# tudelft-iv/CCVPE

Hardware: AMD Instinct MI355X
Metric: image-pairs/sec (higher is better)
Workload: dtype f32

## Files before the change

ccvpe_amd/_lib.py:

```python
import ctypes
import os
import subprocess

import torch

_HERE = os.path.dirname(os.path.abspath(__file__))
LIB_PATH = os.environ.get("CCVPE_LIB") or os.path.join(_HERE, "libccvpe_hip.so")
CSRC_DIR = os.path.join(_HERE, "csrc")

c_float_p = ctypes.c_void_p
c_int = ctypes.c_int
c_float = ctypes.c_float
c_void_p = ctypes.c_void_p


class ConvDesc(ctypes.Structure):
    _fields_ = [
        ("src0", c_void_p), ("src1", c_void_p), ("gate", c_void_p), ("w", c_void_p),
        ("scale", c_void_p), ("shift", c_void_p), ("residual", c_void_p), ("dst", c_void_p),
        ("c0", c_int), ("ld0", c_int), ("c1", c_int), ("ld1", c_int),
        ("batch", c_int), ("in_h", c_int), ("in_w", c_int),
        ("kh", c_int), ("kw", c_int), ("stride", c_int), ("pad", c_int),
        ("n", c_int), ("kpad", c_int), ("ldd", c_int), ("ldres", c_int),
        ("act", c_int), ("out_mode", c_int),
    ]


class UpconvDesc(ctypes.Structure):
    _fields_ = [
        ("src0", c_void_p), ("src1", c_void_p), ("w", c_void_p), ("shift9", c_void_p), ("dst", c_void_p),
        ("c0", c_int), ("ld0", c_int), ("c1", c_int), ("ld1", c_int),
        ("batch", c_int), ("h1", c_int), ("w1", c_int),
        ("n", c_int), ("kpad", c_int), ("ldd", c_int), ("act", c_int),
    ]


class TailDesc(ctypes.Structure):
    _fields_ = [
        ("x", c_void_p), ("w", c_void_p), ("shift9", c_void_p), ("w2", c_void_p), ("b2", c_void_p), ("out", c_void_p),
        ("batch", c_int), ("h1", c_int), ("w1", c_int),
        ("c0", c_int), ("ld0", c_int), ("kpad", c_int),
        ("cout", c_int), ("normalize", c_int), ("split", c_int), ("softmax_partial", c_void_p),
    ]


PROTOTYPES = {
    "ccvpe_last_error": (ctypes.c_char_p, []),
    "ccvpe_abi_version": (c_int, []),
    "ccvpe_multi_copy_f32": (c_int, [ctypes.POINTER(c_void_p), ctypes.POINTER(c_void_p), ctypes.POINTER(c_int), c_int, c_void_p]),
    "ccvpe_gather_repack_f32": (c_int, [c_void_p, c_void_p, c_void_p, c_void_p, c_void_p, c_int, c_void_p]),
    "ccvpe_gather_repack_chunk": (c_int, []),
    "ccvpe_ctx_create": (c_int, [c_void_p, ctypes.c_longlong, c_void_p, c_void_p, ctypes.POINTER(c_void_p)]),
    "ccvpe_ctx_destroy": (c_int, [c_void_p]),
    "ccvpe_ctx_info": (c_int, [c_void_p] + [ctypes.POINTER(ctypes.c_longlong)] * 4 + [ctypes.POINTER(c_int)] * 2),
    "ccvpe_ctx_output": (c_int, [c_void_p, c_int, ctypes.POINTER(c_void_p), ctypes.POINTER(ctypes.c_longlong),
                                  ctypes.POINTER(c_int), ctypes.POINTER(ctypes.c_longlong), ctypes.POINTER(ctypes.c_longlong)]),
    "ccvpe_forward": (c_int, [c_void_p, c_void_p, c_void_p, ctypes.POINTER(c_void_p), c_void_p]),
    "ccvpe_tail512_partials": (c_int, [ctypes.POINTER(TailDesc), c_int]),
    "ccvpe_softmax_apply_f32": (c_int, [c_void_p, c_void_p, c_int, c_void_p, c_int, c_int, c_void_p]),
    "ccvpe_tail512_f32": (c_int, [ctypes.POINTER(TailDesc), c_void_p]),
    "ccvpe_tail512_bf16": (c_int, [ctypes.POINTER(TailDesc), c_void_p]),
    "ccvpe_conv_igemm_f32": (c_int, [ctypes.POINTER(ConvDesc), c_void_p]),
    "ccvpe_conv_igemm_splitk_floats": (c_int, [ctypes.POINTER(ConvDesc), c_int]),
    "ccvpe_conv_igemm_route": (c_int, [ctypes.POINTER(ConvDesc), c_int, c_int]),
    "ccvpe_set_narrow_kernels": (c_int, [c_int]),
    "ccvpe_set_pw_ring_kernels": (c_int, [c_int]),
    "ccvpe_set_mbconv_plane_kernels": (c_int, [c_int]),
    "ccvpe_mbconv_front_route": (c_int, [c_int] * 8),
    "ccvpe_mbconv_band_plan": (c_int, [c_int] * 7),
    "ccvpe_conv3x3_variant": (c_int, [ctypes.POINTER(ConvDesc), c_int]),
    "ccvpe_set_match_mfma": (c_int, [c_int]),
    "ccvpe_match_route": (c_int, [c_int, c_int, ctypes.POINTER(c_int)] + [c_int] * 10 + [ctypes.POINTER(c_int)]),
    "ccvpe_set_pwn_kernels": (c_int, [c_int]),
    "ccvpe_conv3x3_wino_ok": (c_int, [ctypes.POINTER(ConvDesc)]),
    "ccvpe_conv3x3_wino_f32": (c_int, [ctypes.POINTER(ConvDesc), c_void_p]),
    "ccvpe_conv3x3_match1_ok": (c_int, [ctypes.POINTER(ConvDesc), c_int, c_int]),
    "ccvpe_conv3x3_match1_bf16": (c_int, [ctypes.POINTER(ConvDesc), c_int, c_void_p, c_int, c_int, c_int, c_int, c_int, c_void_p, c_void_p]),
    "ccvpe_conv_igemm_splitk_f32": (c_int, [ctypes.POINTER(ConvDesc), c_void_p, c_void_p]),
    "ccvpe_conv_igemm_splitk_bf16": (c_int, [ctypes.POINTER(ConvDesc), c_int, c_void_p, c_void_p]),
    "ccvpe_upconv3x3_f32": (c_int, [ctypes.POINTER(UpconvDesc), c_void_p]),
    "ccvpe_upconv3x3_bf16": (c_int, [ctypes.POINTER(UpconvDesc), c_void_p]),
    "ccvpe_upconv3x3_route": (c_int, [ctypes.POINTER(UpconvDesc), c_int]),
    "ccvpe_upconv3x3_s3_ok": (c_int, [ctypes.POINTER(UpconvDesc)]),
    "ccvpe_upconv3x3_s3_f32": (c_int, [ctypes.POINTER(UpconvDesc), c_void_p]),
    "ccvpe_upconv3x3_s3_form_ok": (c_int, [ctypes.POINTER(UpconvDesc), c_int]),
    "ccvpe_upconv3x3_s3_route": (c_int, [ctypes.POINTER(UpconvDesc), c_int]),
    "ccvpe_upconv3x3_s3_form_f32": (c_int, [ctypes.POINTER(UpconvDesc), c_int, c_void_p]),
    "ccvpe_set_s3_quad": (c_int, [c_int]),
    "ccvpe_pw_s3_ok": (c_int, [ctypes.POINTER(ConvDesc)]),
    "ccvpe_pw_s3_route": (c_int, [ctypes.POINTER(ConvDesc)]),
    "ccvpe_pw_s3_f32": (c_int, [ctypes.POINTER(ConvDesc), c_void_p]),
    "ccvpe_stem_conv_f32": (c_int, [c_void_p] * 5 + [c_int] * 4 + [c_void_p]),
    "ccvpe_dwconv_nblk": (c_int, [c_int] * 4),
    "ccvpe_dwconv_f32": (c_int, [c_void_p] * 6 + [c_int] * 7 + [c_void_p]),
    "ccvpe_mbconv_front_nblk": (c_int, [c_int] * 6),
    "ccvpe_stem_dw_nblk": (c_int, [c_int] * 3),
    "ccvpe_stem_dw_f32": (c_int, [c_void_p] * 9 + [c_int] * 4 + [c_void_p]),
    "ccvpe_stem_dw_bf16": (c_int, [c_void_p] * 9 + [c_int] * 4 + [c_void_p]),
    "ccvpe_mbconv_front_f32": (c_int, [c_void_p, c_void_p, c_int] + [c_void_p] * 7 + [c_int] * 8 + [c_void_p]),
    "ccvpe_mbconv_front_s3_ok": (c_int, [c_int] * 7),
    "ccvpe_mbconv_front_s3_f32": (c_int, [c_void_p, c_void_p, c_int] + [c_void_p] * 7 + [c_int] * 8 + [c_void_p]),
    "ccvpe_se_gate_f32": (c_int, [c_void_p, c_int, c_float] + [c_void_p] * 5 + [c_int] * 3 + [c_void_p]),
    "ccvpe_ground_descriptor_f32": (c_int, [c_void_p, c_int, c_void_p, c_void_p, ctypes.POINTER(c_int),
                                            c_void_p, c_int, c_int, c_int, c_void_p]),
    "ccvpe_match_level_f32": (c_int, [c_void_p, c_int, c_void_p, c_int, c_int, ctypes.POINTER(c_int),
                                      c_int, c_int, c_int, c_int, c_int, c_void_p, c_void_p, c_int, c_int,
                                      c_int, c_int, c_void_p]),
    "ccvpe_head_conv3x3_f32": (c_int, [c_void_p] * 4 + [c_int] * 5 + [c_void_p]),
    "ccvpe_cast_bf16_f32": (c_int, [c_void_p, c_void_p, ctypes.c_long, c_void_p]),
    "ccvpe_softmax_rows_f32": (c_int, [c_void_p, c_void_p, c_int, c_int, c_void_p]),
    "ccvpe_eval_postprocess_f32": (c_int, [c_void_p, c_void_p, c_void_p, c_int, c_int, c_int, c_void_p]),
    "ccvpe_eval_metrics_f32": (c_int, [c_void_p] * 7 + [c_int, c_int, c_int, c_void_p]),
    "ccvpe_belief_partials": (c_int, [c_int, c_int]),
    "ccvpe_belief_step_f32": (c_int, [c_void_p] * 5 + [c_int, c_float] + [c_void_p] * 4 + [c_int] * 3 + [c_void_p]),
    "ccvpe_infonce_scratch_floats": (c_int, [c_int, c_int]),
    "ccvpe_infonce_loss_f32": (c_int, [c_void_p, c_void_p, c_float, c_void_p, c_void_p, c_void_p, c_int, c_int, c_void_p]),
    "ccvpe_cross_entropy_loss_f32": (c_int, [c_void_p] * 4 + [c_int, c_int, c_void_p]),
    "ccvpe_orientation_loss_f32": (c_int, [c_void_p] * 5 + [c_int, c_int, c_void_p]),
    "ccvpe_stem_conv_raw_f32": (c_int, [c_void_p] * 3 + [c_int] * 4 + [c_void_p]),
    "ccvpe_dwconv_raw_f32": (c_int, [c_void_p] * 3 + [c_int] * 7 + [c_void_p]),
    "ccvpe_bn_stats_nblk": (c_int, [c_int]),
    "ccvpe_bn_stats_f32": (c_int, [c_void_p, c_int, c_int] + [c_void_p] * 4 + [c_float, c_void_p, c_void_p]),
    "ccvpe_bn_act_nblk": (c_int, [c_int]),
    "ccvpe_bn_act_f32": (c_int, [c_void_p] * 5 + [c_float, c_int] + [c_void_p] * 4 + [c_int] * 3 + [c_void_p]),
    "ccvpe_conv_wgrad_tile": (c_int, [c_int, c_int]),
    "ccvpe_conv_wgrad_scratch_floats": (c_int, [c_int] * 9),
    "ccvpe_conv_wgrad_f32": (c_int, [c_void_p, c_int, c_int, c_void_p, c_int, c_int, c_void_p, c_int, c_void_p,
                                     c_void_p] + [c_int] * 8 + [c_void_p]),
    "ccvpe_conv_wgrad_gated_f32": (c_int, [c_void_p, c_int, c_int, c_void_p, c_void_p, c_int, c_void_p, c_void_p, c_int, c_int, c_int,
                                           c_int, c_void_p]),
    "ccvpe_conv_wgrad_bias_f32": (c_int, [c_void_p, c_int, c_int, c_void_p, c_int, c_int, c_void_p, c_int, c_void_p,
                                          c_void_p, c_void_p] + [c_int] * 8 + [c_void_p]),
    "ccvpe_colsum_f32": (c_int, [c_void_p, c_int, c_int, c_int, c_void_p, c_void_p, c_void_p]),
    "ccvpe_bn_bwd_nblk": (c_int, [c_int]),
    "ccvpe_bn_act_bwd_f32": (c_int, [c_void_p] * 9 + [c_float, c_int] + [c_void_p] * 4 + [c_int] * 3 + [c_void_p]),
    "ccvpe_bn_act_bwd_frozen_f32": (c_int, [c_void_p] * 9 + [c_float, c_int] + [c_void_p] * 4 + [c_int] * 3 + [c_void_p]),
    "ccvpe_se_bn_bwd_reduce_f32": (c_int, [c_void_p] * 6 + [c_float, c_int, c_void_p, c_void_p, c_int, c_int, c_int, c_void_p]),
    "ccvpe_se_bn_bwd_apply_f32": (c_int, [c_void_p] * 8 + [c_float, c_int, c_void_p, c_void_p, c_void_p, c_void_p, c_int, c_int, c_int,
                                          c_void_p]),
    "ccvpe_se_dgate_f32": (c_int, [c_void_p] * 6 + [c_float, c_int, c_void_p] + [c_int] * 3 + [c_void_p]),
    "ccvpe_se_bwd_f32": (c_int, [c_void_p, c_int, c_float, c_void_p, c_int] + [c_void_p] * 10 + [c_int] * 3 + [c_void_p]),
    "ccvpe_dwconv_dgrad_f32": (c_int, [c_void_p] * 3 + [c_int] * 7 + [c_void_p]),
    "ccvpe_dwconv_wgrad_nblk": (c_int, [c_int] * 4),
    "ccvpe_dwconv_wgrad_f32": (c_int, [c_void_p] * 4 + [c_int] * 7 + [c_void_p]),
    "ccvpe_relu_bwd_f32": (c_int, [c_void_p] * 3 + [c_int, c_void_p]),
    "ccvpe_gate_mul_f32": (c_int, [c_void_p] * 3 + [c_int] * 3 + [c_void_p]),
    "ccvpe_softmax_bwd_f32": (c_int, [c_void_p] * 4 + [c_int, c_int, c_void_p]),
    "ccvpe_l2norm2_bwd_f32": (c_int, [c_void_p] * 3 + [c_int, c_int, c_void_p]),
    "ccvpe_head_conv3x3_bwd_f32": (c_int, [c_void_p] * 7 + [c_int] * 5 + [c_void_p]),
    "ccvpe_ground_descriptor_bwd_f32": (c_int, [c_void_p, c_int, c_void_p, ctypes.POINTER(c_int)] + [c_void_p] * 4 +
                                        [c_int] * 3 + [c_void_p]),
    "ccvpe_add_cols_f32": (c_int, [c_void_p, c_int, c_int, c_void_p, c_int, c_int, c_int, c_int, c_void_p]),
    "ccvpe_stem_wgrad_nblk": (c_int, [c_int] * 3),
    "ccvpe_stem_conv_wgrad_f32": (c_int, [c_void_p] * 4 + [c_int] * 4 + [c_void_p]),
    "ccvpe_match_bwd_nblk": (c_int, [c_int, c_int, c_int]),
    "ccvpe_match_level_bwd_f32": (c_int, [c_void_p, c_int, c_void_p, c_int, c_int, ctypes.POINTER(c_int), c_int, c_int,
                                          c_int, c_int, c_int, c_void_p, c_void_p, c_void_p, c_int, c_void_p, c_int, c_void_p,
                                          c_int, c_void_p, c_int, c_int, c_int, c_void_p]),
    "ccvpe_infonce_loss_bwd_f32": (c_int, [c_void_p, c_void_p, c_float, c_void_p, c_void_p, c_void_p, c_int, c_int, c_void_p]),
    "ccvpe_cross_entropy_loss_bwd_f32": (c_int, [c_void_p] * 4 + [c_int, c_int, c_void_p]),
    "ccvpe_orientation_loss_bwd_f32": (c_int, [c_void_p] * 5 + [c_int, c_int, c_void_p]),
    "ccvpe_train_targets_nblk": (c_int, [c_int, c_int]),
    "ccvpe_train_targets_f32": (c_int, [c_void_p, c_void_p, c_int, c_float] + [c_void_p] * 10 + [c_int] * 3 + [c_void_p]),
    "ccvpe_train_targets_ordered_f32": (c_int, [c_void_p, c_void_p, c_int, c_int, c_float] + [c_void_p] * 10 + [c_int] * 3 + [c_void_p]),
    "ccvpe_adam_chunk_elems": (c_int, []),
    "ccvpe_adam_hyper_floats": (c_int, []),
    "ccvpe_adam_step_f32": (c_int, [c_void_p, c_void_p, c_void_p, c_void_p, c_int, c_float, c_void_p]),
    "ccvpe_adam_device_layout": (c_int, [c_int]),
    "ccvpe_grad_sqnorm_f32": (c_int, [c_void_p, c_void_p, c_void_p, c_int, c_float, c_void_p, c_void_p]),
    "ccvpe_adam_prepare_f32": (c_int, [c_void_p, c_void_p, c_void_p, c_void_p, c_int, c_void_p, c_int, c_float, c_void_p, c_void_p]),
    "ccvpe_adam_update_f32": (c_int, [c_void_p, c_void_p, c_void_p, c_void_p, c_int, c_float, c_void_p, c_void_p]),
    "ccvpe_preprocess_u8_f32": (c_int, [c_void_p, c_int, c_int, c_void_p, c_void_p, c_int, c_void_p, c_void_p, c_int, c_void_p,
                                        c_void_p, c_int, c_int, c_int, c_int, ctypes.POINTER(c_float), ctypes.POINTER(c_float),
                                        c_void_p]),
    "ccvpe_resize_u8": (c_int, [c_void_p, c_int, c_int, c_void_p, c_void_p, c_int, c_void_p, c_void_p, c_int, c_void_p, c_void_p,
                                c_int, c_int, c_void_p]),
    "ccvpe_gather_norm_u8_f32": (c_int, [c_void_p, c_void_p, c_int, c_int, c_int, c_int, ctypes.POINTER(c_float),
                                         ctypes.POINTER(c_float), c_void_p, c_void_p]),
    "ccvpe_window_resize_norm_u8_f32": (c_int, [c_void_p, c_int, c_int, c_void_p, c_int, c_int, c_int, c_void_p, c_void_p, c_int,
                                                c_void_p, c_void_p, c_int, ctypes.POINTER(c_float), ctypes.POINTER(c_float),
                                                c_void_p, c_int, c_int, c_void_p]),
    "ccvpe_kitti_align_u8": (c_int, [c_void_p, ctypes.c_long, c_void_p, c_void_p, c_int, c_void_p, c_int, c_int, c_void_p]),
    "ccvpe_kitti_align_norm_u8_f32": (c_int, [c_void_p, c_void_p, c_int, ctypes.POINTER(c_float), ctypes.POINTER(c_float),
                                              c_void_p, c_int, c_int, c_void_p]),
    "ccvpe_conv_igemm_bf16": (c_int, [ctypes.POINTER(ConvDesc), c_int, c_void_p]),
    "ccvpe_stem_conv_bf16": (c_int, [c_void_p] * 5 + [c_int] * 4 + [c_void_p]),
    "ccvpe_dwconv_bf16": (c_int, [c_void_p] * 6 + [c_int] * 7 + [c_void_p]),
    "ccvpe_mbconv_front_bf16": (c_int, [c_void_p, c_void_p, c_int] + [c_void_p] * 7 + [c_int] * 8 + [c_void_p]),
    "ccvpe_match_level_bf16": (c_int, [c_void_p, c_int, c_void_p, c_int, c_int, ctypes.POINTER(c_int),
                                       c_int, c_int, c_int, c_int, c_int, c_void_p, c_void_p, c_int, c_int,
                                       c_int, c_int, c_void_p]),
    "ccvpe_head_conv3x3_bf16": (c_int, [c_void_p] * 4 + [c_int] * 5 + [c_void_p]),
}

_lib = None
weights_epoch = 0


def build(verbose=False):
    cmd = ["make", "-C", CSRC_DIR, "-j8"]
    res = subprocess.run(cmd, capture_output=True, text=True)
    if verbose or res.returncode != 0:
        print(res.stdout)
        print(res.stderr)
    if res.returncode != 0:
        raise RuntimeError("building libccvpe_hip.so failed (see output above)")
    return LIB_PATH


def load():
    global _lib
    if _lib is not None:
        return _lib
    if not os.path.isfile(LIB_PATH):
        raise RuntimeError(
            "libccvpe_hip.so not found at %s — run `python -c 'import __graft_entry__ as g; g.build()'` "
            "(or `make -C ccvpe_amd/csrc`).  ccvpe_amd has no CPU fallback." % LIB_PATH)
    lib = ctypes.CDLL(LIB_PATH)
    lax = bool(os.environ.get("CCVPE_LIB")) and os.environ.get("CCVPE_LIB_ALLOW_MISSING") == "1"
    for name, (res, args) in PROTOTYPES.items():
        if lax and not hasattr(lib, name):
            continue
        fn = getattr(lib, name)
        fn.restype = res
        fn.argtypes = args
    if os.environ.get("CCVPE_NARROW") == "0" and hasattr(lib, "ccvpe_set_narrow_kernels"):
        lib.ccvpe_set_narrow_kernels(0)
    if os.environ.get("CCVPE_PW_RING") == "0" and hasattr(lib, "ccvpe_set_pw_ring_kernels"):
        lib.ccvpe_set_pw_ring_kernels(0)
    if os.environ.get("CCVPE_MATCH_MFMA") == "0" and hasattr(lib, "ccvpe_set_match_mfma"):
        lib.ccvpe_set_match_mfma(0)
    if os.environ.get("CCVPE_PWN") == "0" and hasattr(lib, "ccvpe_set_pwn_kernels"):
        lib.ccvpe_set_pwn_kernels(0)
    if os.environ.get("CCVPE_S3_QUAD") == "0" and hasattr(lib, "ccvpe_set_s3_quad"):
        lib.ccvpe_set_s3_quad(0)
    if os.environ.get("CCVPE_MBPLANE") is not None and hasattr(lib, "ccvpe_set_mbconv_plane_kernels"):
        lib.ccvpe_set_mbconv_plane_kernels(int(os.environ["CCVPE_MBPLANE"]))
    _lib = lib
    return lib


class CcvpeError(RuntimeError):
    pass


def check(status, what):
    if status != 0:
        msg = load().ccvpe_last_error()
        raise CcvpeError("%s failed (%d): %s" % (what, status, msg.decode() if msg else "?"))
```

ccvpe_amd/csrc/conv3x3_wino.hip:

```cpp
#include "conv_common.h"

namespace ccvpe {

static constexpr int WG_NW = 4;
static constexpr int WG_NT = 2;
static constexpr int WG_BN = 16 * WG_NT;
static constexpr int WG_XS = 8;
static constexpr int WG_TH = 4 * WG_NW;
static constexpr int WG_HR = WG_TH + 2, WG_HC = 18;
static constexpr int WG_HPX = WG_HR * WG_HC;
static constexpr int WG_HS = WG_HPX * LDS_LD;
static constexpr int WG_BS = 2 * WG_XS * WG_BN * 16;
static constexpr int WG_LDS = (WG_HS + WG_BS) * 4;

__global__ __launch_bounds__(256, 2) void conv3x3_wino_kernel(const IgemmParams p) {
  constexpr int NTHR = 64 * WG_NW;
  constexpr int H_IT = (WG_HPX * 4 + NTHR - 1) / NTHR;
  extern __shared__ __attribute__((aligned(16))) float wg_sm[];
  float* Hs = wg_sm;
  float* Bs = wg_sm + WG_HS;

  const int tid = threadIdx.x;
  const int lane = tid & 63;
  const int wave = sgpr(tid >> 6);
// ... 33 lines not shown
  int h_chunk = 0;
  const int ld0s = sgpr(p.ld0);
  auto load_halo = [&](int chunk) {
    h_chunk = chunk;
#pragma unroll
    for (int it = 0; it < H_IT; ++it) {
      const int ch = chunk * 16 + h_sub[it] * 4;
      const bool ok = h_pix[it] >= 0 && ch < ctot;
      const size_t off = ok ? (size_t)h_pix[it] * ld0s + ch : 0;
      h_reg[it] = *reinterpret_cast<const f32x4*>(src0 + off);
    }
  };
  auto store_halo = [&]() {
#pragma unroll
    for (int it = 0; it < H_IT; ++it)
      if (h_off[it] >= 0)
        *reinterpret_cast<f32x4*>(Hs + h_off[it]) = keep_if(h_reg[it], h_pix[it] >= 0 && h_chunk * 16 + h_sub[it] * 4 < ctot);
  };

  const int rl = lane >> 2;
  const int grp = wave & 1;
  const unsigned wvoff = ((unsigned)(n0 + grp * 16 + rl) * (unsigned)p.Kpad + (unsigned)(((lane & 3) ^ w_swz(rl)) * 4)) * 4u;
  const unsigned bs_lds = (unsigned)(uintptr_t)(__attribute__((address_space(3))) float*)Bs;
  auto load_w = [&](int chunk, int g, int dbuf) {
#pragma unroll
    for (int q = 0; q < 4; ++q) {
      const int t = (wave >> 1) + 2 * q;
      const char* sbase = reinterpret_cast<const char*>(wp) + ((size_t)(g * WG_XS + t) * cpad + (size_t)chunk * 16) * 4;
      const unsigned lds = __builtin_amdgcn_readfirstlane(bs_lds + (unsigned)(((dbuf * WG_XS + t) * WG_BN + grp * 16) * 16 * 4));
      asm volatile("s_mov_b32 m0, %0\n\tglobal_load_lds_dwordx4 %1, %2" ::"s"(lds), "v"(wvoff), "s"(sbase) : "memory", "m0");
    }
  };
  auto dma_wait = [&]() { asm volatile("s_waitcnt vmcnt(0)" ::: "memory"); };

  f32x4 acc[16][WG_NT];
#pragma unroll
  for (int x = 0; x < 16; ++x)
#pragma unroll
    for (int j = 0; j < WG_NT; ++j) acc[x][j] = (f32x4){0.f, 0.f, 0.f, 0.f};

  const int frow = lane & 15;
  const int fk = (lane >> 4) * 4;
  const int bcol = ((lane >> 4) ^ w_swz(frow)) * 4;
  const int ttx = frow & 7, tty = frow >> 3;
  const int dbase = ((4 * wave + 2 * tty) * WG_HC + 2 * ttx) * LDS_LD + fk;

  load_halo(0);
  load_w(0, 0, 0);
  store_halo();
  dma_wait();
  __syncthreads();

  int chunk = 0;
  auto stage = [&](int s, auto gtag) {
    constexpr int G = decltype(gtag)::value;
    const bool more = s + 1 < nstages;
    if (G == 0 && chunk + 1 < nchunks) load_halo(chunk + 1);
    if (more) load_w(G == 1 ? chunk + 1 : chunk, G ^ 1, (s + 1) & 1);

    f32x4 d[3][4];
#pragma unroll
    for (int r = 0; r < 3; ++r)
#pragma unroll
      for (int x = 0; x < 4; ++x) d[r][x] = *reinterpret_cast<const f32x4*>(Hs + dbase + ((G + r) * WG_HC + x) * LDS_LD);
    f32x4 v[2][4];
#pragma unroll
    for (int x = 0; x < 4; ++x) {
      const f32x4 t0 = G == 0 ? d[0][x] - d[2][x] : d[1][x] - d[0][x];
      const f32x4 t1 = G == 0 ? d[1][x] + d[2][x] : d[0][x] - d[2][x];
      if (x == 0) { v[0][0] = t0; v[1][0] = t1; }
      else if (x == 1) { v[0][1] = t0; v[1][1] = t1; }
      else if (x == 2) { v[0][2] = t0; v[1][2] = t1; }
      else { v[0][3] = t0; v[1][3] = t1; }
    }
#pragma unroll
    for (int rr = 0; rr < 2; ++rr) {
      const f32x4 a0 = v[rr][0], a1 = v[rr][1], a2 = v[rr][2], a3 = v[rr][3];
      v[rr][0] = a0 - a2;
      v[rr][1] = a1 + a2;
      v[rr][2] = a2 - a1;
      v[rr][3] = a1 - a3;
    }
    __builtin_amdgcn_sched_barrier(0);
#pragma unroll
    for (int t = 0; t < WG_XS; ++t) {
      f32x4 bf[WG_NT];
#pragma unroll
      for (int j = 0; j < WG_NT; ++j)
        bf[j] = *reinterpret_cast<const f32x4*>(&Bs[(((s & 1) * WG_XS + t) * WG_BN + j * 16 + frow) * 16 + bcol]);
      const f32x4 vv = v[t >> 2][t & 3];
#pragma unroll
      for (int kk = 0; kk < 4; ++kk)
#pragma unroll
        for (int j = 0; j < WG_NT; ++j)
          acc[G * WG_XS + t][j] = __builtin_amdgcn_mfma_f32_16x16x4f32(bf[j][kk], vv[kk], acc[G * WG_XS + t][j], 0, 0, 0);
    }
    __builtin_amdgcn_sched_barrier(0);
    dma_wait();
    __syncthreads();
    if (G == 1 && more) {
      store_halo();
      __syncthreads();
    }
  };
  for (int s = 0; s < nstages; s += 2, ++chunk) {
    stage(s, std::integral_constant<int, 0>{});
    stage(s + 1, std::integral_constant<int, 1>{});
  }

  const int oy = y0 + 4 * wave + 2 * tty, ox = x0 + 2 * ttx;
  if (oy >= p.H || ox >= p.W) return;
  float* dst = reinterpret_cast<float*>(p.dst);
  const size_t m00 = (size_t)(b * p.H + oy) * p.W + ox;
#pragma unroll
  for (int j = 0; j < WG_NT; ++j) {
    const int n = n0 + j * 16 + fk;
    if (n >= p.N) continue;
    f32x4 y[2][2];
#pragma unroll
    for (int r = 0; r < 4; ++r) {
      float m[4][4];
#pragma unroll
      for (int x = 0; x < 16; ++x) m[x >> 2][x & 3] = acc[x][j][r];
      float q0[4], q1[4];
#pragma unroll
      for (int c = 0; c < 4; ++c) {
        q0[c] = m[0][c] + m[1][c] + m[2][c];
        q1[c] = m[1][c] - m[2][c] - m[3][c];
      }
      const float bias = (p.shift && n + r < p.N) ? p.shift[n + r] : 0.0f;
      y[0][0][r] = q0[0] + q0[1] + q0[2] + bias;
      y[0][1][r] = q0[1] - q0[2] - q0[3] + bias;
      y[1][0][r] = q1[0] + q1[1] + q1[2] + bias;
      y[1][1][r] = q1[1] - q1[2] - q1[3] + bias;
    }
#pragma unroll
    for (int dy = 0; dy < 2; ++dy)
#pragma unroll
      for (int dx = 0; dx < 2; ++dx) {
        const size_t o = (m00 + (size_t)dy * p.W + dx) * p.ldd + n;
        if (n + 3 < p.N) {
          *reinterpret_cast<f32x4*>(dst + o) = y[dy][dx];
        } else {
#pragma unroll
          for (int r = 0; r < 4; ++r)
            if (n + r < p.N) dst[o + r] = y[dy][dx][r];
        }
      }
  }
}

static int round_up(int v, int m) { return (v + m - 1) / m * m; }

static const char* wino_refusal(const ccvpe_conv_desc* d) {
  if (!d) return "null desc";
  if (d->kh != 3 || d->kw != 3 || d->stride != 1 || d->pad != 1 || d->out_mode != CCVPE_OUT_NHWC) return "3x3 / stride 1 / pad 1 / NHWC only";
  if (d->c1 != 0 || d->src1 || d->gate || d->scale || d->residual || d->act != CCVPE_ACT_NONE)
    return "one source, bias only (no gate, scale, residual or activation)";
  if (d->in_h <= 0 || d->in_w <= 0 || d->in_h % 2 || d->in_w % 2) return "H and W must be even";
  if (d->c0 < 32 || d->c0 % 4 || d->ld0 < d->c0 || d->ld0 % 4) return "c0 >= 32, c0 and ld0 multiples of 4";
  if (d->n <= 0 || d->ldd < d->n || d->ldd % 4) return "ldd >= n, ldd multiple of 4";
  if (d->kpad != 16 * round_up(d->c0, 16)) return "kpad must be 16 * round_up(c0, 16) (packed U)";
  if ((long)d->batch * d->in_h * d->in_w < 16384) return "fewer than 16384 output pixels";
  if ((long)d->batch * d->in_h * d->in_w > 0x7fffffffL) return "too many pixels";
  if ((size_t)round_up(d->n, WG_BN) * d->kpad * 4 >= (1ull << 32)) return "U larger than 4 GB";
  if (!aligned16(d->src0) || !aligned16(d->w) || !aligned16(d->dst)) return "pointers must be 16-byte aligned";
  ccvpe_conv_desc dd = *d;
  dd.kpad = round_up(9 * d->c0, 16);
  if (ccvpe_conv_igemm_splitk_floats(&dd, 0) != 0) return "the direct path splits K at this shape";
  return nullptr;
}

}

using namespace ccvpe;

extern "C" int ccvpe_conv3x3_wino_ok(const ccvpe_conv_desc* d) { return wino_refusal(d) ? 0 : 1; }

extern "C" int ccvpe_conv3x3_wino_f32(const ccvpe_conv_desc* d, void* stream) {
  if (const char* why = wino_refusal(d)) return fail(CCVPE_EINVAL, "conv3x3_wino: %s", why);
  IgemmParams p{};
  p.src0 = d->src0; p.w = d->w; p.shift = d->shift; p.dst = d->dst;
  p.c0 = d->c0; p.ld0 = d->ld0;
  p.H = d->in_h; p.W = d->in_w;
  p.N = d->n; p.Kpad = d->kpad; p.Npad = round_up(d->n, WG_BN);
  p.ldd = d->ldd;
  p.tiles_x = (p.W + 15) / 16;
  p.tiles_y = (p.H + WG_TH - 1) / WG_TH;
  p.tiles_n = p.Npad / WG_BN;
  const long total = (long)p.tiles_x * p.tiles_y * d->batch * p.tiles_n;
  if (total > 0x7fffffffL) return fail(CCVPE_EINVAL, "conv3x3_wino: grid too large");
  p.tiles_total = (int)total;
  static DevCache lds_set;
  if (int rc = ensure_dyn_lds(lds_set, conv3x3_wino_kernel, WG_LDS, "conv3x3_wino")) return rc;
  hipLaunchKernelGGL(conv3x3_wino_kernel, dim3(p.tiles_total), dim3(64 * WG_NW), WG_LDS, (hipStream_t)stream, p);
  return check_launch("conv3x3_wino_kernel");
}
```

ccvpe_amd/csrc/conv_common.h:

```cpp
#pragma once
#include "common.h"
#include <cstdlib>
#include <type_traits>

namespace ccvpe {

typedef float f32x4 __attribute__((ext_vector_type(4)));
typedef __bf16 bf16_t;
typedef __bf16 bf16x8 __attribute__((ext_vector_type(8)));
typedef __bf16 bf16x4 __attribute__((ext_vector_type(4)));

template <typename T> struct ElemTraits;
template <> struct ElemTraits<float> { static constexpr int E = 4; };
template <> struct ElemTraits<bf16_t> { static constexpr int E = 8; };

template <typename T>
__device__ __forceinline__ f32x4 mfma_stage(f32x4 wfrag, f32x4 afrag, f32x4 acc);
template <>
__device__ __forceinline__ f32x4 mfma_stage<float>(f32x4 wfrag, f32x4 afrag, f32x4 acc) {
#pragma unroll
  for (int kk = 0; kk < 4; ++kk) acc = __builtin_amdgcn_mfma_f32_16x16x4f32(wfrag[kk], afrag[kk], acc, 0, 0, 0);
  return acc;
}
template <>
// ... 32 lines not shown
template <typename T>
__device__ __forceinline__ f32x4 gate_apply(f32x4 raw, f32x4 g0, f32x4 g1) {
  if (sizeof(T) == 4) return raw * g0;
  bf16x8 v = __builtin_bit_cast(bf16x8, raw);
  bf16x8 o;
#pragma unroll
  for (int i = 0; i < 4; ++i) {
    o[i] = (bf16_t)((float)v[i] * g0[i]);
    o[i + 4] = (bf16_t)((float)v[i + 4] * g1[i]);
  }
  return __builtin_bit_cast(f32x4, o);
}
__device__ __forceinline__ int sgpr(int v) { return __builtin_amdgcn_readfirstlane(v); }

struct IgemmParams {
  const void* src0;
  const void* src1;
  const float* gate;
  const void* w;
  const float* scale;
  const float* shift;
  const void* residual;
  void* dst;
  int out_f32;
  int c0, ld0, c1, ld1;
  int H, W, Ho, Wo;
  int kw, stride, pad;
  int N, Kpad, Npad;
  int cpt0, cpt, total_chunks, stages;
  int ldd, ldres, act, out_mode, cout;
  int M;
  long in_pixels;
  int tiles_n, tiles_total;
  int tiles_x, tiles_y;
  int ksplit, sps;
  float* partial;
  int ablate;
};

constexpr int LDS_LD = 20;
template <typename T> struct PanelLayout {
  static constexpr bool SWZ = true;
  static constexpr int LD = SWZ ? 16 : LDS_LD;
};
__device__ __forceinline__ int panel_swz(int row) { return ((row >> 2) & 1) << 1; }

__device__ __forceinline__ int xcd_tile(int bid, int total) {
  const int q = total / 8, r = total % 8;
  const int xcd = bid % 8, loc = bid / 8;
  return (xcd < r ? xcd * (q + 1) : r * (q + 1) + (xcd - r) * q) + loc;
}

template <typename T, int ACT>
__device__ __forceinline__ void store4(const IgemmParams& p, f32x4 v, int n, size_t obase, size_t rbase,
                                       const float* sc, const float* sh) {
#pragma unroll
  for (int r = 0; r < 4; ++r) {
    float t = v[r] * sc[r] + sh[r];
    if (ACT == CCVPE_ACT_RELU) t = fmaxf(t, 0.0f);
    else if (ACT == CCVPE_ACT_SWISH) t = swishf(t);
    v[r] = t;
  }
  const T* res = reinterpret_cast<const T*>(p.residual);
  const bool f32out = sizeof(T) == 4 || p.out_f32;
  if (n + 3 < p.N) {
    if (res) {
      f32x4 rf;
      if (sizeof(T) == 4) {
        rf = *reinterpret_cast<const f32x4*>(res + rbase + n);
      } else {
        const bf16x4 rv = *reinterpret_cast<const bf16x4*>(res + rbase + n);
#pragma unroll
        for (int r = 0; r < 4; ++r) rf[r] = (float)rv[r];
      }
      if (ACT == CCVPE_ACT_RELU_MASK) {
#pragma unroll
        for (int r = 0; r < 4; ++r) v[r] = rf[r] > 0.f ? v[r] : 0.f;
      } else {
        v += rf;
      }
    }
    if (f32out) {
      *reinterpret_cast<f32x4*>(reinterpret_cast<float*>(p.dst) + obase) = v;
    } else {
      bf16x4 o;
#pragma unroll
      for (int r = 0; r < 4; ++r) o[r] = (bf16_t)v[r];
      *reinterpret_cast<bf16x4*>(reinterpret_cast<bf16_t*>(p.dst) + obase) = o;
    }
  } else {
#pragma unroll
    for (int r = 0; r < 4; ++r)
      if (n + r < p.N) {
        float t = v[r];
        if (res) {
          const float rf = (float)res[rbase + n + r];
          t = ACT == CCVPE_ACT_RELU_MASK ? (rf > 0.f ? t : 0.f) : t + rf;
        }
        if (f32out) reinterpret_cast<float*>(p.dst)[obase + r] = t;
        else reinterpret_cast<bf16_t*>(p.dst)[obase + r] = (bf16_t)t;
      }
  }
}

#define CCVPE_ACT_DISPATCH(act, body)                                            \
  do {                                                                           \
    if ((act) == CCVPE_ACT_SWISH) body(std::integral_constant<int, CCVPE_ACT_SWISH>{});      \
    else if ((act) == CCVPE_ACT_RELU) body(std::integral_constant<int, CCVPE_ACT_RELU>{});   \
    else if ((act) == CCVPE_ACT_RELU_MASK) body(std::integral_constant<int, CCVPE_ACT_RELU_MASK>{}); \
    else body(std::integral_constant<int, CCVPE_ACT_NONE>{});                    \
  } while (0)

__device__ __forceinline__ int w_swz(int r) { return (0x1320 >> (((r >> 2) & 3) * 4)) & 3; }

#define CCVPE_TILES(X)                                                            \
  X(4, 5, 2) X(4, 4, 2) X(4, 3, 2) X(4, 2, 2) X(4, 1, 2)  \
  X(4, 5, 1) X(4, 3, 1) X(4, 1, 1)                        \
  X(2, 7, 1)

struct TileCfg { int mt, nt, wn; };
#define CCVPE_TILE_ROW(MT_, NT_, WN_) {MT_, NT_, WN_},
static const TileCfg kCfgs[] = {CCVPE_TILES(CCVPE_TILE_ROW)};
#undef CCVPE_TILE_ROW

static int pick_cfg(int npad16) {
  int best = 0;
  long best_cost = -1;
  for (int i = 0; i < (int)(sizeof(kCfgs) / sizeof(kCfgs[0])); ++i) {
    const int bn = 16 * kCfgs[i].nt * kCfgs[i].wn;
    const int tiles = (npad16 + bn - 1) / bn;
    const long cost = (long)tiles * bn * 1000 + (1000 - bn);
    if (best_cost < 0 || cost < best_cost) { best_cost = cost; best = i; }
  }
  return best;
}


template <typename T> int pw_dispatch(const IgemmParams& p, int mt, int nt, int wn, hipStream_t stream);
template <typename T> int conv3x3_dispatch(const IgemmParams& p, int batch, int mt, int nt, int wn, hipStream_t stream);
template <typename T> int conv3x3_variant_query(const IgemmParams& p, int batch, int mt, int nt, int wn);
extern bool g_use_pw2;
template <typename T> bool pw2_supported(const IgemmParams& p, int mt, int nt, int wn);
template <typename T> int pw2_dispatch(const IgemmParams& p, int mt, int nt, int wn, hipStream_t stream);
extern bool g_use_narrow;
int c3n_supported(const IgemmParams& p, int batch);
int c3n_dispatch(const IgemmParams& p, int batch, hipStream_t stream);
int c3n_match_supported(const IgemmParams& p, int batch, int L);
int c3n_match_dispatch(const IgemmParams& p, int batch, const float* g, int ldg, int L, int off, float* scores, hipStream_t stream);
extern bool g_use_pwn;
bool pwn_supported(const IgemmParams& p, int batch, int esz);
int pwn_dispatch(const IgemmParams& p, int batch, int esz, hipStream_t stream);
int up2_supported(int c0, int c1, int n, int kpad, int h1, int w1, int batch);
int up2_launch(int id, const ccvpe_upconv_desc* d, hipStream_t stream);
bool upconv_s3q_serves(const ccvpe_upconv_desc* d);
int upconv_s3q_launch(const ccvpe_upconv_desc* d, hipStream_t stream);

template <typename P>
static void s3_fill(const ccvpe_upconv_desc* d, P& p) {
  p.src0 = reinterpret_cast<const float*>(d->src0); p.src1 = reinterpret_cast<const float*>(d->src1);
  p.w = d->w; p.shift9 = d->shift9; p.dst = reinterpret_cast<float*>(d->dst);
  p.c0 = d->c0; p.ld0 = d->ld0; p.c1 = d->c1; p.ld1 = d->ld1;
  p.H1 = d->h1; p.W1 = d->w1; p.batch = d->batch; p.N = d->n; p.ldd = d->ldd; p.act = d->act;
  p.nb0 = (d->c0 + 15) / 16; p.nb1 = (d->c1 + 15) / 16; p.nst = 4 * p.nb0 + 9 * p.nb1;
}

}
```

ccvpe_amd/csrc/plan.hip:

```cpp
#include <cstring>
#include <string>
#include <unordered_map>
#include <utility>
#include <vector>

#include "common.h"

namespace ccvpe {

enum : uint32_t { K_INT = 0, K_FLT = 1, K_NULL = 2, K_WEIGHTS = 3, K_WORKSPACE = 4, K_GRD = 5, K_SAT = 6, K_STREAM = 7, K_BLOB = 8 };

template <typename A> struct FromSlot {
  static A get(uint64_t v) { return (A)(int64_t)v; }
};
template <typename P> struct FromSlot<P*> {
  static P* get(uint64_t v) { return reinterpret_cast<P*>((uintptr_t)v); }
};
template <> struct FromSlot<float> {
  static float get(uint64_t v) { uint32_t b = (uint32_t)v; float f; std::memcpy(&f, &b, 4); return f; }
};
template <typename... A, size_t... I>
static int invoke_seq(int (*f)(A...), const uint64_t* v, std::index_sequence<I...>) { return f(FromSlot<A>::get(v[I])...); }
template <typename... A>
static int invoke(int (*f)(A...), const uint64_t* v, int n) {
  if (n != (int)sizeof...(A)) return fail(CCVPE_EINVAL, "plan: call has %d arguments, the entry point takes %d", n, (int)sizeof...(A));
  return invoke_seq(f, v, std::index_sequence_for<A...>{});
}
typedef int (*Invoker)(const uint64_t*, int);

#define CCVPE_REG(fn) {#fn, [](const uint64_t* v, int n) -> int { return invoke(fn, v, n); }}
static const std::unordered_map<std::string, Invoker>& registry() {
  static const std::unordered_map<std::string, Invoker> r = {
      CCVPE_REG(ccvpe_conv_igemm_f32), CCVPE_REG(ccvpe_conv_igemm_bf16), CCVPE_REG(ccvpe_conv_igemm_splitk_f32),
      CCVPE_REG(ccvpe_conv_igemm_splitk_bf16), CCVPE_REG(ccvpe_conv3x3_match1_bf16), CCVPE_REG(ccvpe_conv3x3_wino_f32),
      CCVPE_REG(ccvpe_upconv3x3_f32), CCVPE_REG(ccvpe_upconv3x3_bf16), CCVPE_REG(ccvpe_upconv3x3_s3_f32), CCVPE_REG(ccvpe_pw_s3_f32),
      CCVPE_REG(ccvpe_tail512_f32), CCVPE_REG(ccvpe_tail512_bf16), CCVPE_REG(ccvpe_stem_conv_f32), CCVPE_REG(ccvpe_stem_conv_bf16),
      CCVPE_REG(ccvpe_stem_dw_f32), CCVPE_REG(ccvpe_stem_dw_bf16),
      CCVPE_REG(ccvpe_dwconv_f32), CCVPE_REG(ccvpe_dwconv_bf16), CCVPE_REG(ccvpe_mbconv_front_f32), CCVPE_REG(ccvpe_mbconv_front_bf16),
      CCVPE_REG(ccvpe_mbconv_front_s3_f32),
      CCVPE_REG(ccvpe_se_gate_f32), CCVPE_REG(ccvpe_ground_descriptor_f32), CCVPE_REG(ccvpe_match_level_f32),
      CCVPE_REG(ccvpe_match_level_bf16), CCVPE_REG(ccvpe_head_conv3x3_f32), CCVPE_REG(ccvpe_head_conv3x3_bf16),
      CCVPE_REG(ccvpe_softmax_rows_f32), CCVPE_REG(ccvpe_softmax_apply_f32), CCVPE_REG(ccvpe_cast_bf16_f32), CCVPE_REG(ccvpe_eval_postprocess_f32),
  };
  return r;
}
#undef CCVPE_REG

struct Patch { uint32_t call, arg, kind; uint64_t off; };
struct BlobPatch { uint32_t blob, field, kind; uint64_t off; };
struct Call { Invoker fn; std::string name; uint32_t first, nargs, sid; int wait_on; };
struct Output { uint64_t off, bytes; uint32_t dtype, ndim; long long dims[4], strides[4]; };

}

struct ccvpe_ctx {
  std::vector<ccvpe::Call> calls;
  std::vector<uint64_t> args;
  std::vector<std::vector<unsigned char>> blobs;
  std::vector<ccvpe::Patch> patches;
  std::vector<ccvpe::BlobPatch> blob_patches;
  std::vector<ccvpe::Output> outputs;
  uint64_t workspace_bytes = 0, weights_bytes = 0, grd_bytes = 0, sat_bytes = 0;
  char* weights = nullptr;
  char* workspace = nullptr;
  bool own_weights = false, own_workspace = false;
  hipStream_t side = nullptr;
  std::vector<hipEvent_t> events;
};

using namespace ccvpe;

namespace {
struct Reader {
  const unsigned char* p;
  const unsigned char* end;
  bool ok = true;
  template <typename T> T get() {
    T v{};
    if (sizeof(T) > (size_t)(end - p)) { ok = false; return v; }
    std::memcpy(&v, p, sizeof(T));
    p += sizeof(T);
    return v;
  }
  const unsigned char* bytes(size_t n) {
    if (n > (size_t)(end - p)) { ok = false; return nullptr; }
    const unsigned char* q = p;
    p += n;
    return q;
  }
};
}

extern "C" int ccvpe_ctx_create(const void* plan, long long n_bytes, void* weights_dev, void* workspace_dev, ccvpe_ctx** out) {
  if (!plan || n_bytes < 64 || !out) return fail(CCVPE_EINVAL, "ctx_create: null / short plan");
  Reader r{reinterpret_cast<const unsigned char*>(plan), reinterpret_cast<const unsigned char*>(plan) + n_bytes};
  const unsigned char* magic = r.bytes(8);
  if (!magic || std::memcmp(magic, "CCVPLAN1", 8)) return fail(CCVPE_EINVAL, "ctx_create: not a CCVPE plan (bad magic)");
  ccvpe_ctx* c = new ccvpe_ctx();
  auto bail = [&](int code, const char* msg) { delete c; return fail(code, "ctx_create: %s", msg); };
  const int abi = (int)r.get<uint32_t>();
  const uint32_t flags = r.get<uint32_t>();
  (void)flags;
  if (abi != ccvpe_abi_version()) {
    delete c;
    return fail(CCVPE_EINVAL, "ctx_create: the plan was recorded against ABI %d, this library is ABI %d", abi, ccvpe_abi_version());
  }
  c->workspace_bytes = r.get<uint64_t>();
  c->weights_bytes = r.get<uint64_t>();
  c->grd_bytes = r.get<uint64_t>();
  c->sat_bytes = r.get<uint64_t>();
  const uint32_t n_calls = r.get<uint32_t>(), n_blobs = r.get<uint32_t>(), n_out = r.get<uint32_t>();
  r.get<uint32_t>();
  if (!r.ok || n_calls > (1u << 20) || n_blobs > (1u << 20) || n_out > 64) return bail(CCVPE_EINVAL, "corrupt header");
  for (uint32_t i = 0; i < n_out; ++i) {
    Output o;
    o.off = r.get<uint64_t>(); o.bytes = r.get<uint64_t>(); o.dtype = r.get<uint32_t>(); o.ndim = r.get<uint32_t>();
    for (int k = 0; k < 4; ++k) o.dims[k] = (long long)r.get<uint64_t>();
    for (int k = 0; k < 4; ++k) o.strides[k] = (long long)r.get<uint64_t>();
    if (o.off > c->workspace_bytes || o.bytes > c->workspace_bytes - o.off) return bail(CCVPE_EINVAL, "output outside the workspace");
    c->outputs.push_back(o);
  }
  struct Reloc { uint32_t blob, field, kind; uint64_t value; };
  std::vector<Reloc> relocs;
  for (uint32_t i = 0; i < n_blobs && r.ok; ++i) {
    const uint32_t nb = r.get<uint32_t>(), nr = r.get<uint32_t>();
    for (uint32_t k = 0; k < nr; ++k) {
      Reloc q{i, r.get<uint32_t>(), r.get<uint32_t>(), r.get<uint64_t>()};
      if ((uint64_t)q.field + 8 > (uint64_t)nb) return bail(CCVPE_EINVAL, "relocation outside its blob");
      relocs.push_back(q);
    }
    const unsigned char* d = r.bytes((nb + 7) & ~7u);
    if (!d) return bail(CCVPE_EINVAL, "truncated blob");
    c->blobs.emplace_back(d, d + nb);
  }
  struct RawArg { uint32_t kind; uint64_t value; };
  std::vector<std::vector<RawArg>> raw(n_calls);
  for (uint32_t i = 0; i < n_calls && r.ok; ++i) {
    const unsigned char* nm = r.bytes(48);
    if (!nm) break;
    std::string name(reinterpret_cast<const char*>(nm), strnlen(reinterpret_cast<const char*>(nm), 48));
    const uint32_t na = r.get<uint32_t>();
    const uint32_t sid = r.get<uint32_t>() & 1u;
    if (na > 64) return bail(CCVPE_EINVAL, "call with more than 64 arguments");
    for (uint32_t k = 0; k < na; ++k) {
      RawArg a{r.get<uint32_t>(), 0};
      r.get<uint32_t>();
      a.value = r.get<uint64_t>();
      raw[i].push_back(a);
    }
    if (name == "@wait") {
      if (na != 2) return bail(CCVPE_EINVAL, "malformed stream wait");
      c->calls.push_back(Call{nullptr, name, 0, 0, (uint32_t)(raw[i][0].value & 1), (int)(raw[i][1].value & 1)});
      raw[i].clear();
      continue;
    }
    auto it = registry().find(name);
    if (it == registry().end()) {
      delete c;
      return fail(CCVPE_EINVAL, "ctx_create: the plan calls %s, which this library does not replay", name.c_str());
    }
    c->calls.push_back(Call{it->second, name, 0, na, sid, -1});
  }
  if (!r.ok) return bail(CCVPE_EINVAL, "truncated plan");
  size_t woff = (size_t)(r.p - reinterpret_cast<const unsigned char*>(plan));
  woff = (woff + 255) & ~(size_t)255;
  if (woff > (size_t)n_bytes || c->weights_bytes > (uint64_t)((size_t)n_bytes - woff)) return bail(CCVPE_EINVAL, "truncated weights");
  if (weights_dev) c->weights = reinterpret_cast<char*>(weights_dev);
  else {
    if (hipMalloc(reinterpret_cast<void**>(&c->weights), c->weights_bytes ? c->weights_bytes : 256) != hipSuccess) return bail(CCVPE_ELAUNCH, "hipMalloc(weights)");
    c->own_weights = true;
  }
  if (workspace_dev) c->workspace = reinterpret_cast<char*>(workspace_dev);
  else {
    if (hipMalloc(reinterpret_cast<void**>(&c->workspace), c->workspace_bytes ? c->workspace_bytes : 256) != hipSuccess) {
      if (c->own_weights) (void)hipFree(c->weights);
      return bail(CCVPE_ELAUNCH, "hipMalloc(workspace)");
    }
    c->own_workspace = true;
  }
  if (c->weights_bytes &&
      hipMemcpy(c->weights, reinterpret_cast<const unsigned char*>(plan) + woff, c->weights_bytes, hipMemcpyHostToDevice) != hipSuccess) {
    ccvpe_ctx_destroy(c);
    return fail(CCVPE_ELAUNCH, "ctx_create: weight upload failed");
  }
  auto resolve = [&](uint32_t kind, uint64_t v, bool& dynamic, bool& bad) -> uint64_t {
    dynamic = bad = false;
    switch (kind) {
// ... 108 lines not shown
```

ccvpe_amd/models.py:

```python
import torch
import torch.nn as nn

from . import ops
from .synth import B0_BLOCKS, MODEL_SPECS, state_dict_spec

BN_EPS = 1e-3
SKIP_BLOCKS = (15, 10, 4, 2, 0)
MATCH_STRIDES = {"vigor": (64, 32, 16, 8, 4, 2),
                 "kitti": (128, 64, 32, 16, 8, 8),
                 "oxford": (64, 32, 16, 8, 4, 2)}


def window_offset(kind, channels, length):
    return int(channels / 2 - length / 2) if kind == "oxford" else 0


def _round_up(v, m):
    return (v + m - 1) // m * m


class _Holder(nn.Module):

    def forward(self, *a, **k):
        raise RuntimeError("parameter holder is not callable; use the owning CVM_* module")


def _populate(root, kind, init):
    for key, shape, role in state_dict_spec(kind):
        parts = key.split(".")
        node = root
        for name in parts[:-1]:
            child = node._modules.get(name)
            if child is None:
                child = _Holder()
                node.add_module(name, child)
            node = child
        t = init[key].clone()
        if role in ("bn_m", "bn_v", "bn_n"):
            node.register_buffer(parts[-1], t)
        else:
            node.register_parameter(parts[-1], nn.Parameter(t))


def _pad2(w, dtype=torch.float32, n_mult=16):
    k_mult = 16 if dtype == torch.float32 else 32
    n, k = w.shape
    if n % n_mult == 0 and k % k_mult == 0:
        out = w.to(dtype).contiguous()
        return out.clone() if out.data_ptr() == w.data_ptr() else out
    out = w.new_zeros((_round_up(n, n_mult), _round_up(k, k_mult)))
    out[:n, :k] = w
    return out.to(dtype).contiguous()


def _pack_conv(w, dtype=torch.float32):
    o = w.shape[0]
    return _pad2(w.permute(0, 2, 3, 1).reshape(o, -1), dtype)


_WINO_G = ((1.0, 0.0, 0.0), (0.5, 0.5, 0.5), (0.5, -0.5, 0.5), (0.0, 0.0, 1.0))


def _pack_wino(w, dtype=torch.float32):
    if dtype != torch.float32:
        return None
    o, i = w.shape[0], w.shape[1]
    g = torch.tensor(_WINO_G, dtype=torch.float64, device=w.device)
    u = torch.einsum("ak,ockl,bl->oabc", g, w.to(torch.float64), g)
    out = torch.zeros((_round_up(o, 32), 4, 4, _round_up(i, 16)), dtype=torch.float64, device=w.device)
    out[:o, :, :, :i] = u
    return out.reshape(out.shape[0], -1).to(torch.float32).contiguous()


def _fold_bn(sd, p):
    scale = sd[p + ".weight"] / torch.sqrt(sd[p + ".running_var"] + BN_EPS)
    shift = sd[p + ".bias"] - sd[p + ".running_mean"] * scale
    return scale.contiguous(), shift.contiguous()


class _Obj(object):
    pass


def _pack_pw_s3(w):
    if w is None or w.dtype != torch.float32 or w.dim() != 2 or w.shape[1] % 16 or w.shape[0] % 16:
        return None
    npad, k = w.shape
    return torch.cat(_split3_bf16(w.reshape(npad, k // 16, 16).permute(1, 0, 2)), -1).contiguous()


def _unpack_pw_s3(w3):
    nst, npad, _ = w3.shape
    return tuple(w3[..., 16 * q:16 * q + 16].float().permute(1, 0, 2).reshape(npad, nst * 16) for q in range(3))


PW_S3_MIN_MID = 240


MB_S3_MAX_CIN = 48


def _pack_encoder(sd, p, dtype=torch.float32, fold_bn=True, s3=False):
    fold = _fold_bn if fold_bn else (lambda _sd, _p: (None, None))
    e = _Obj()
    e.stem_w = sd[p + "._conv_stem.weight"].permute(2, 3, 1, 0).contiguous()
    e.stem_scale, e.stem_shift = fold(sd, p + "._bn0")
    e.blocks = []
    for i, (k, s, ex, cin, cout) in enumerate(B0_BLOCKS):
        b = _Obj()
        bp = "%s._blocks.%d" % (p, i)
        b.k, b.s, b.expand, b.cin, b.cout, b.mid = k, s, ex != 1, cin, cout, cin * ex
        if b.expand:
            b.w_exp = _pack_conv(sd[bp + "._expand_conv.weight"], dtype)
            b.s0, b.b0 = fold(sd, bp + "._bn0")
            b.w_exp3 = _pack_pw_s3(b.w_exp) if s3 and cin <= MB_S3_MAX_CIN else None
        b.w_dw = sd[bp + "._depthwise_conv.weight"].reshape(b.mid, k, k).permute(1, 2, 0).contiguous()
        b.s1, b.b1 = fold(sd, bp + "._bn1")
        b.se_w1 = sd[bp + "._se_reduce.weight"].reshape(-1, b.mid).contiguous()
        b.se_b1 = sd[bp + "._se_reduce.bias"].contiguous()
        b.se_w2 = sd[bp + "._se_expand.weight"].reshape(b.mid, -1).t().contiguous()
        b.se_b2 = sd[bp + "._se_expand.bias"].contiguous()
        b.w_proj = _pack_conv(sd[bp + "._project_conv.weight"], dtype)
        b.w_proj3 = _pack_pw_s3(b.w_proj) if s3 and b.mid >= PW_S3_MIN_MID else None
        b.s2, b.b2 = fold(sd, bp + "._bn2")
        b.skip = (s == 1 and cin == cout)
        e.blocks.append(b)
    e.w_head = _pack_conv(sd[p + "._conv_head.weight"], dtype)
    e.w_head3 = _pack_pw_s3(e.w_head) if s3 else None
    e.head_scale, e.head_shift = fold(sd, p + "._bn1")
    return e


def _pack_deconv(w, bias, col_map, ldo, dtype=torch.float32):
    cin, cout = w.shape[0], w.shape[1]
    wg = w.permute(2, 3, 1, 0).reshape(4 * cout, cin)
    out = w.new_zeros((4 * cout, ldo))
    for d0, s0, n in col_map:
        out[:, d0:d0 + n] = wg[:, s0:s0 + n]
    return _pad2(out, dtype), bias.repeat(4).contiguous()


_UP_S = {0: {0: ((0, 1),), 1: ((1, 0), (2, 1))}, 1: {0: ((0, 0), (1, 1)), 1: ((2, 0),)}}
_UP_R = {0: (1, 2), 1: (0, 1, 2), 2: (0, 1)}
_OVERLAP_ENV = __import__("os").environ.get("CCVPE_OVERLAP_DECODERS", "auto")


OVERLAP_DECODERS_MAX_BATCH = 128


def _overlap_decoders(precision, batch=1):
    return _OVERLAP_ENV == "1" or (_OVERLAP_ENV == "auto" and precision == "bf16" and batch <= OVERLAP_DECODERS_MAX_BATCH)
FOLD_LEVELS = tuple(int(c) for c in __import__("os").environ.get("CCVPE_FOLD_LEVELS", "012345"))
FOLD_MIN_PIXELS = int(__import__("os").environ.get("CCVPE_FOLD_MIN_PIXELS", "2048"))
FUSE_TAIL = __import__("os").environ.get("CCVPE_FUSE_TAIL", "1") != "0"
SPLIT_TAIL = __import__("os").environ.get("CCVPE_SPLIT_TAIL", "1") != "0"
WINO = __import__("os").environ.get("CCVPE_WINO", "1") != "0"
SPLIT3 = __import__("os").environ.get("CCVPE_SPLIT3", "1") != "0"
SPLIT3_TAIL = SPLIT3 and __import__("os").environ.get("CCVPE_SPLIT3_TAIL", "1") != "0"
SPLIT3_MIN_OK = 2
SPLIT3_PW = SPLIT3 and __import__("os").environ.get("CCVPE_SPLIT3_PW", "1") != "0"
SPLIT3_PW_MIN_OK = 2
SPLIT3_MB = SPLIT3 and __import__("os").environ.get("CCVPE_SPLIT3_MB", "1") != "0"
SPLIT3_MB_MIN_OK = 2
PACK_GRAPH = __import__("os").environ.get("CCVPE_PACK_GRAPH", "1") != "0"
PACK_GATHER = __import__("os").environ.get("CCVPE_PACK_GATHER", "1") != "0"
FUSE_MATCH = __import__("os").environ.get("CCVPE_FUSE_MATCH", "1") != "0"
FUSE_STEM = __import__("os").environ.get("CCVPE_FUSE_STEM", "1") != "0"
EVAL_TWO_STREAMS = __import__("os").environ.get("CCVPE_EVAL_TWO_STREAMS", "1") != "0"


def _tail_split(precision, x, cout):
    if x.dtype != torch.float32:
        return 0
    if precision == "bf16":
        return 1 if SPLIT_TAIL and cout == 1 else 0
    return 2 if SPLIT3 and SPLIT3_TAIL else 0


def _pack_upconv(wd, bd, col_map, cp, w3, b3, dtype=torch.float32):
    cd, co = wd.shape[1], w3.shape[0]
    c1 = w3.shape[1] - cd
    wd_my = wd.new_zeros((cp, cd, 2, 2), dtype=torch.float64)
    for d0, s0, n in col_map:
        wd_my[d0:d0 + n] = wd[s0:s0 + n].double()
    w3d = w3[:, :cd].double()
    k = 4 * cp + 9 * c1
    kmult = 16 if dtype == torch.float32 else 32
    out = wd.new_zeros((4, _round_up(co, 16), _round_up(k, kmult)), dtype=torch.float64)
    for py in range(2):
        for px in range(2):
            par = py * 2 + px
            for du in range(2):
                for dv in range(2):
                    weff = wd.new_zeros((co, cp), dtype=torch.float64)
                    for ky, a in _UP_S[py][du]:
                        for kx, b in _UP_S[px][dv]:
                            weff += w3d[:, :, ky, kx] @ wd_my[:, :, a, b].t()
                    tap = du * 2 + dv
                    out[par, :co, tap * cp:(tap + 1) * cp] = weff
            if c1:
                out[par, :co, 4 * cp:k] = w3[:, cd:].double().permute(0, 2, 3, 1).reshape(co, 9 * c1)
    shift9 = wd.new_zeros((9, co), dtype=torch.float64)
    for rc in range(3):
        for cc in range(3):
            v = b3.double().clone()
            for ky in _UP_R[rc]:
                for kx in _UP_R[cc]:
                    v += w3d[:, :, ky, kx] @ bd.double()
            shift9[rc * 3 + cc] = v
    return out.to(dtype).contiguous(), shift9.float().contiguous()


def _split3_bf16(v):
    hi = v.to(torch.bfloat16)
    r = v - hi.float()
    mid = r.to(torch.bfloat16)
    lo = (r - mid.float()).to(torch.bfloat16)
    return hi, mid, lo


def _pack_upconv_s3(fw, cp, c1, dtype=torch.float32):
    if dtype != torch.float32 or fw is None or fw.dtype != torch.float32 or c1 <= 0:
        return None
    npad = fw.shape[1]
    nb0, nb1 = (cp + 15) // 16, (c1 + 15) // 16
    a = fw.new_zeros((4, npad, 4, nb0 * 16))
    a[..., :cp] = fw[:, :, :4 * cp].reshape(4, npad, 4, cp)
    a = a.reshape(4, npad, 4, nb0, 16).permute(0, 3, 2, 1, 4).reshape(4, 4 * nb0, npad, 16)
    s = fw.new_zeros((4, npad, 9, nb1 * 16))
    s[..., :c1] = fw[:, :, 4 * cp:4 * cp + 9 * c1].reshape(4, npad, 9, c1)
    s = s.reshape(4, npad, 9, nb1, 16).permute(0, 2, 3, 1, 4).reshape(4, 9 * nb1, npad, 16)
    return torch.cat(_split3_bf16(torch.cat([a, s], 1)), -1).contiguous()


def _pack_backward(sd, kind, pk):
    spec = MODEL_SPECS[kind]
    n_rot = spec["n_rot"]
    bwd = {}
    for enc in ("grd_efficientnet", "sat_efficientnet"):
        for i, (k, s_, ex, cin, cout) in enumerate(B0_BLOCKS):
            bp = "%s._blocks.%d" % (enc, i)
            if ex != 1:
                bwd[bp + "._expand_conv.weight"] = _pack_conv(sd[bp + "._expand_conv.weight"].permute(1, 0, 2, 3))
            bwd[bp + "._project_conv.weight"] = _pack_conv(sd[bp + "._project_conv.weight"].permute(1, 0, 2, 3))
            if s_ == 1:
                mid = cin * ex
                w_dw = sd[bp + "._depthwise_conv.weight"].reshape(mid, k * k).t()
                bwd[bp + "._depthwise_conv.weight"] = w_dw.flip(0).contiguous()
        bwd[enc + "._conv_head.weight"] = _pack_conv(sd[enc + "._conv_head.weight"].permute(1, 0, 2, 3))
    for j in range(6):
        lvl = 6 - j
        for branch, lv in (("", pk.loc[j]), ("_ori", pk.ori[j])):
            conv, deconv = "conv%d%s" % (lvl, branch), "deconv%d%s" % (lvl, branch)
            if lvl != 1:
                bwd[conv + ".2.weight"] = _pack_conv(sd[conv + ".2.weight"].flip(2, 3).permute(1, 0, 2, 3))
            bwd[conv + ".0.weight"] = _pack_conv(sd[conv + ".0.weight"].flip(2, 3).permute(1, 0, 2, 3))
            w_ref = sd[deconv + ".weight"]
            if branch == "":
                c = lv.c
                k_rows, cmap = lv.ldo, [(0, 1, c), (c, 0, 1)]
            elif j == 0:
                c6 = spec["ori"][0][0] - n_rot
                k_rows, cmap = lv.k, [(0, n_rot, c6), (c6 + 1, 0, n_rot)]
            else:
                k_rows, cmap = lv.k, [(0, 0, spec["ori"][j][0])]
            w_ours = w_ref.new_zeros((k_rows,) + tuple(w_ref.shape[1:]))
            for d0, s0, n in cmap:
                w_ours[d0:d0 + n] = w_ref[s0:s0 + n]
            bwd[deconv + ".weight"] = _pack_conv(w_ours)
    w = sd["sat_feature_to_descriptors.1.weight"]
    w4 = w.view(w.shape[0], 1280, 2, 2)
    bwd["sat_feature_to_descriptors.1.weight"] = _pack_deconv(w4, w4.new_zeros((1280,)), [(0, 0, w.shape[0])], w.shape[0])[0]
    wcat = torch.cat([sd["grd_feature_to_descriptor%d.0.weight" % l] for l in range(1, 7)], 0)
    ld = _round_up(pk.gd_n, 4)
    wpad = wcat.new_zeros((ld,) + tuple(wcat.shape[1:]))
    wpad[:pk.gd_n] = wcat
    bwd["grd_feature_to_descriptor.0.weight"] = _pack_conv(wpad.permute(1, 0, 2, 3))
    return bwd


def _pack_model(sd, kind, n_tail, dtype=torch.float32, fold=True, f32_tail=0):
    spec = MODEL_SPECS[kind]
    pk = _Obj()
    pk.dtype = dtype
    pk.f32_from = 6 - f32_tail if dtype != torch.float32 else 6
    base_dtype = dtype
    s3 = fold and dtype == torch.float32
    pk.grd = _pack_encoder(sd, "grd_efficientnet", dtype, fold_bn=fold, s3=s3)
    pk.sat = _pack_encoder(sd, "sat_efficientnet", dtype, fold_bn=fold, s3=s3)
    ws, bs, wh, bh = [], [], [], []
    for l in range(1, 7):
        p = "grd_feature_to_descriptor%d" % l
        ws.append(sd[p + ".0.weight"].reshape(-1, 1280))
        bs.append(sd[p + ".0.bias"])
        wh.append(sd[p + ".2.weight"].reshape(-1))
        bh.append(sd[p + ".2.bias"].reshape(-1))
    pk.gd_w = _pad2(torch.cat(ws, 0), dtype)
    pk.gd_w3 = _pack_pw_s3(pk.gd_w) if s3 else None
    pk.gd_bias = torch.cat(bs, 0).contiguous()
    pk.gd_n = pk.gd_bias.shape[0]
    pk.gd_wh = torch.stack(wh, 0).contiguous()
    pk.gd_bh = torch.cat(bh, 0).contiguous()
    w = sd["sat_feature_to_descriptors.1.weight"]
    pk.sd_w = _pack_conv(w.view(w.shape[0], 1280, 2, 2), dtype)
    pk.sd_w3 = _pack_pw_s3(pk.sd_w) if s3 else None
    pk.sd_bias = sd["sat_feature_to_descriptors.1.bias"].contiguous()
    pk.sd_n = w.shape[0]

    pk.loc, pk.ori = [], []
    n_rot = spec["n_rot"]
    for j in range(6):
        lvl = 6 - j
        dc_in, dc_out, c_in, c_out = spec["loc"][j]
        dtype = torch.float32 if j >= pk.f32_from else base_dtype
        c = dc_in - 1
        ldo = _round_up(c + 1 + (n_tail if j == 0 else 0), 8)
        lv = _Obj()
        lv.c, lv.ldo, lv.up_n = c, ldo, 4 * dc_out
        lv.up_w, lv.up_b = _pack_deconv(sd["deconv%d.weight" % lvl], sd["deconv%d.bias" % lvl],
                                        [(0, 1, c), (c, 0, 1)], ldo, dtype)
        lv.c0, lv.c1 = dc_out, c_in - dc_out
        lv.n_a = c_out
        if fold and j in FOLD_LEVELS:
            lv.fw, lv.fshift = _pack_upconv(sd["deconv%d.weight" % lvl], sd["deconv%d.bias" % lvl],
                                            [(0, 1, c), (c, 0, 1)], ldo, sd["conv%d.0.weight" % lvl],
                                            sd["conv%d.0.bias" % lvl], dtype)
            lv.fw3 = _pack_upconv_s3(lv.fw, ldo, lv.c1, dtype if base_dtype == torch.float32 else None)
        lv.w_a = _pack_conv(sd["conv%d.0.weight" % lvl], dtype)
        lv.b_a = sd["conv%d.0.bias" % lvl].contiguous()
        if lvl != 1:
            lv.w_b = _pack_conv(sd["conv%d.2.weight" % lvl], dtype)
            lv.u_b = _pack_wino(sd["conv%d.2.weight" % lvl], base_dtype) if fold else None
            lv.n_b = c_out
        else:
            lv.w_b = sd["conv1.2.weight"].permute(0, 2, 3, 1).contiguous()
        lv.b_b = sd["conv%d.2.bias" % lvl].contiguous()
        pk.loc.append(lv)
        dtype = base_dtype
        dc_in, dc_out, c_in, c_out = spec["ori"][j]
        ov = _Obj()
        if j == 0:
            c6 = dc_in - n_rot
            ov.k = pk.loc[0].ldo
            ov.k_algo = dc_in
            ov.up_w, ov.up_b = _pack_deconv(sd["deconv6_ori.weight"], sd["deconv6_ori.bias"],
                                            [(0, n_rot, c6), (c6 + 1, 0, n_rot)], pk.loc[0].ldo, dtype)
        else:
            ov.k = ov.k_algo = dc_in
            ov.up_w, ov.up_b = _pack_deconv(sd["deconv%d_ori.weight" % lvl], sd["deconv%d_ori.bias" % lvl],
                                            [(0, 0, dc_in)], dc_in, dtype)
        ov.up_n = 4 * dc_out
        ov.c0, ov.c1 = dc_out, c_in - dc_out
        if fold and j in FOLD_LEVELS:
            cmap = [(0, n_rot, c6), (c6 + 1, 0, n_rot)] if j == 0 else [(0, 0, dc_in)]
            ov.fw, ov.fshift = _pack_upconv(sd["deconv%d_ori.weight" % lvl], sd["deconv%d_ori.bias" % lvl], cmap,
                                            ov.k, sd["conv%d_ori.0.weight" % lvl], sd["conv%d_ori.0.bias" % lvl],
                                            dtype)
            ov.fw3 = _pack_upconv_s3(ov.fw, ov.k, ov.c1, dtype)
        ov.w_a = _pack_conv(sd["conv%d_ori.0.weight" % lvl], dtype)
        ov.b_a = sd["conv%d_ori.0.bias" % lvl].contiguous()
        ov.n_a = c_out
        if lvl != 1:
            ov.w_b = _pack_conv(sd["conv%d_ori.2.weight" % lvl], dtype)
            ov.u_b = _pack_wino(sd["conv%d_ori.2.weight" % lvl], dtype) if fold else None
            ov.n_b = c_out
        else:
            ov.w_b = sd["conv1_ori.2.weight"].permute(0, 2, 3, 1).contiguous()
        ov.b_b = sd["conv%d_ori.2.bias" % lvl].contiguous()
        pk.ori.append(ov)
    pk.bwd = _pack_backward(sd, kind, pk) if (not fold and base_dtype == torch.float32) else None
    return pk


def _pw(x, c0, w, w3, n, *, batch, in_h, in_w, two=False, gate=None, scale=None, shift=None, residual=None, act=ops.ACT_NONE,
        ldd=None, out_f32=False):
    if (SPLIT3 and SPLIT3_PW and w3 is not None and x.dtype == torch.float32 and
            ops.pw_s3_ok(x, c0, w3, n, batch=batch, in_h=in_h, in_w=in_w, two=two, gate=gate, residual=residual, act=act,
                         ldd=ldd) >= SPLIT3_PW_MIN_OK):
        return ops.pw_s3(x, c0, w3, n, batch=batch, in_h=in_h, in_w=in_w, two=two, gate=gate, scale=scale, shift=shift,
                         residual=residual, act=act, ldd=ldd)
    kk = dict(kh=2, kw=2, stride=2) if two else {}
    return ops.conv_igemm(x, c0, w, n, batch=batch, in_h=in_h, in_w=in_w, gate=gate, scale=scale, shift=shift, residual=residual,
                          act=act, ldd=ldd, out_f32=out_f32, **kk)


def _run_encoder(e, img, circular, multiscale, dtype=torch.float32):
    blk0 = e.blocks[0]
    stem_fused = (FUSE_STEM and not blk0.expand and blk0.k == 3 and blk0.s == 1 and blk0.mid == 32
                  and ops.stem_dw_supported(img.shape[2], img.shape[3], circular) > 0)
    x = None if stem_fused else ops.stem_conv(img, e.stem_w, e.stem_scale, e.stem_shift, circular, out_dtype=dtype)
    feats = []
    for blk in e.blocks:
        if x is not None:
            b, h, w, _ = x.shape
        if x is None:
            u, part = ops.stem_dw(img, e.stem_w, e.stem_scale, e.stem_shift, blk.w_dw, blk.s1, blk.b1, circular,
                                  out_dtype=dtype)
            b = u.shape[0]
        elif blk.expand and ops.mbconv_front_supported(h, w, blk.cin, blk.mid, blk.k, blk.s):
            w3 = getattr(blk, "w_exp3", None)
            if SPLIT3 and SPLIT3_MB and w3 is not None and ops.mbconv_front_s3_ok(x, w3, blk.mid, blk.k, blk.s) >= SPLIT3_MB_MIN_OK:
                u, part = ops.mbconv_front_s3(x, w3, blk.s0, blk.b0, blk.w_dw, blk.s1, blk.b1, blk.mid, blk.k, blk.s, circular)
            else:
                u, part = ops.mbconv_front(x, blk.w_exp, blk.s0, blk.b0, blk.w_dw, blk.s1, blk.b1, blk.mid,
                                           blk.k, blk.s, circular)
        else:
            t = x
            if blk.expand:
                t = ops.conv_igemm(x, blk.cin, blk.w_exp, blk.mid, batch=b, in_h=h, in_w=w,
                                   scale=blk.s0, shift=blk.b0, act=ops.ACT_SWISH)
            u, part = ops.dwconv(t, blk.w_dw, blk.s1, blk.b1, blk.k, blk.s, circular)
        ho, wo = u.shape[1], u.shape[2]
        gate = ops.se_gate(part, ho * wo, blk.se_w1, blk.se_b1, blk.se_w2, blk.se_b2)
        x = _pw(u, blk.mid, blk.w_proj, getattr(blk, "w_proj3", None), blk.cout, batch=b, in_h=ho, in_w=wo, gate=gate,
                scale=blk.s2, shift=blk.b2, residual=x if blk.skip else None)
        if multiscale:
            feats.append(x)
    b, h, w, _ = x.shape
    f = _pw(x, 320, e.w_head, getattr(e, "w_head3", None), 1280, batch=b, in_h=h, in_w=w, scale=e.head_scale,
            shift=e.head_shift, act=ops.ACT_SWISH)
    return f, feats


def _double_conv(lv, up, skip, batch, hw):
    y = ops.conv_igemm(up, lv.c0, lv.w_a, lv.n_a, batch=batch, in_h=hw, in_w=hw, kh=3, kw=3, pad=1,
                       src1=skip, c1=lv.c1, shift=lv.b_a, act=ops.ACT_RELU)
    return y


def _conv_b(lv, y, batch, hw, out_f32=False):
    if (WINO and lv.u_b is not None and
            ops.conv3x3_wino_ok(y, lv.n_a, lv.u_b, lv.n_b, batch=batch, in_h=hw, in_w=hw)):
        return ops.conv3x3_wino(y, lv.n_a, lv.u_b, lv.n_b, batch=batch, in_h=hw, in_w=hw, shift=lv.b_b)
    return ops.conv_igemm(y, lv.n_a, lv.w_b, lv.n_b, batch=batch, in_h=hw, in_w=hw, kh=3, kw=3, pad=1, shift=lv.b_b,
                          out_f32=out_f32)


def _upconv_a(lv, x, k, batch, hw, skip):
    fw3 = getattr(lv, "fw3", None)
    if (SPLIT3 and fw3 is not None and
            ops.upconv3x3_s3_ok(x, k, fw3, lv.n_a, batch=batch, h1=hw, w1=hw, src1=skip, c1=lv.c1) >= SPLIT3_MIN_OK):
        return ops.upconv3x3_s3(x, k, fw3, lv.fshift, lv.n_a, batch=batch, h1=hw, w1=hw, src1=skip, c1=lv.c1, act=ops.ACT_RELU)
    return ops.upconv3x3(x, k, lv.fw, lv.fshift, lv.n_a, batch=batch, h1=hw, w1=hw, src1=skip, c1=lv.c1, act=ops.ACT_RELU)


class _CVMBase(nn.Module):
    kind = "vigor"

    def __init__(self, device, circular_padding, ori_noise=None, efficientnet_weights=None):
        super().__init__()
        self.device = device
        self.circular_padding = circular_padding
        self.ori_noise = ori_noise
        from . import init as _init
        _populate(self, self.kind, _init.reference_init_state_dict(self.kind))
        weights = efficientnet_weights if efficientnet_weights is not None else __import__("os").environ.get("CCVPE_EFFICIENTNET_B0")
        if weights:
            _init.load_efficientnet_b0(self, weights)
        self._pack_cache = None
        self._pack_key = None
        self.precision = "fp32"
        self.fp32_tail_levels = 1

    def set_precision(self, precision, fp32_tail_levels=1):
        if precision not in ("fp32", "bf16"):
            raise ValueError("precision must be 'fp32' or 'bf16'")
        if not 0 <= int(fp32_tail_levels) <= 5:
            raise ValueError("fp32_tail_levels must be in 0..5 (level 6 feeds the bf16 orientation decoder)")
        self.precision = precision
        self.fp32_tail_levels = int(fp32_tail_levels)
        return self

    def invalidate(self):
        self._pack_cache = None
        self._pack_key = None
        object.__setattr__(self, "_flat_tensors", None)
        return self

    def _weights_key(self):
        from . import _lib
        flat = getattr(self, "_flat_tensors", None)
        if flat is None:
            flat = list(self.parameters()) + list(self.buffers())
            object.__setattr__(self, "_flat_tensors", flat)
        return (_lib.weights_epoch,) + tuple((t.data_ptr(), t._version) for t in flat)

    def _packed(self):
        epoch = 0 if self.training else getattr(self, "_stats_epoch", 0)
        key = (self.precision, self.fp32_tail_levels, self.training, epoch) + self._weights_key()
        if self._pack_cache is not None and key == self._pack_key:
            return self._pack_cache
        dev = next(self.parameters()).device
        if dev.type != "cuda":
            raise RuntimeError("ccvpe_amd: move the model to the MI355X first (.to('cuda'))")
        sd = {k: v.detach() for k, v in self.state_dict().items()}
        n_tail = MODEL_SPECS[self.kind]["n_rot"]
        dtype = torch.float32 if self.precision == "fp32" else torch.bfloat16

        def pack(src=sd):
            with torch.no_grad():
                return _pack_model(src, self.kind, n_tail, dtype, fold=not self.training, f32_tail=self.fp32_tail_levels)

        if self.training and PACK_GATHER and dtype == torch.float32 and not getattr(self, "_pack_plan_failed", False):
            from . import repack
            where = tuple(t.data_ptr() for t in list(self.parameters()) + list(self.buffers()))
            gp = getattr(self, "_pack_plan", None)
            if gp is not None and gp[0] == where:
                self._pack_cache = gp[1].run()
            else:
                plan = repack.build(sd, pack)
                if plan is None:
                    self._pack_plan, self._pack_plan_failed = None, True
                    return self._packed()
                self._pack_plan = (where, plan)
                self._pack_cache = plan.pk
        elif self.training and PACK_GRAPH:
            where = (self.precision, self.fp32_tail_levels) + tuple(
                t.data_ptr() for t in list(self.parameters()) + list(self.buffers()))
            g = getattr(self, "_pack_graph", None)
            if g is not None and g[0] == where:
                g[1].replay()
                self._pack_cache = g[2]
            elif getattr(self, "_pack_where", None) == where and not getattr(self, "_pack_graph_failed", False):
                try:
                    graph = torch.cuda.CUDAGraph()
                    with torch.cuda.graph(graph, capture_error_mode="thread_local"):
                        pk = pack()
                    graph.replay()
                    self._pack_graph = (where, graph, pk)
                    self._pack_cache = pk
                except Exception:
                    self._pack_graph, self._pack_graph_failed = None, True
                    self._pack_cache = pack()
            else:
                self._pack_graph = None
                self._pack_where = where
                self._pack_cache = pack()
        else:
            self._pack_cache = pack()
        self._pack_key = key
        return self._pack_cache

    def _side_stream(self, which=1):
        dev = next(self.parameters()).device
        streams = self.__dict__.setdefault("_side_streams", {})
        st = streams.get(which)
        if st is None or st.device != dev:
            st = torch.cuda.Stream(device=dev)
            streams[which] = st
        return st

    def _ori_decoder(self, pk, cat6, sfeats, batch):
        xo = cat6
        normalize = not getattr(self, "ori_raw_output", False)
        for j in range(6):
            ov = pk.ori[j]
            hw = xo.shape[1]
            skip = sfeats[SKIP_BLOCKS[j]] if j < 5 else None
            if j == 5 and FUSE_TAIL and j in FOLD_LEVELS and ops.tail512_ok(hw, hw, ov.n_a):
                return ops.tail512(xo, ov.k, ov.fw, ov.fshift, ov.w_b, ov.b_b, 2, normalize, batch=batch, h1=hw, w1=hw,
                                   split=_tail_split(self.precision, xo, 2))
            if j in FOLD_LEVELS and batch * hw * hw >= FOLD_MIN_PIXELS:
                y = _upconv_a(ov, xo, ov.k, batch, hw, skip)
            else:
                up = ops.conv_igemm(xo, ov.k, ov.up_w, ov.up_n, batch=batch, in_h=hw, in_w=hw,
                                    shift=ov.up_b, out_mode=ops.OUT_DECONV2X, algo_k=ov.k_algo)
                y = _double_conv(ov, up, skip, batch, 2 * hw)
            if j < 5:
                xo = _conv_b(ov, y, batch, 2 * hw)
            else:
                return ops.head_conv3x3(y, ov.w_b, ov.b_b, 2, normalize)

    def _loc_shifts(self):
        n_rot = MODEL_SPECS[self.kind]["n_rot"]
        if self.ori_noise is None:
            return list(range(n_rot))
        k = int(self.ori_noise / 18)
        return list(range(-k, k + 1))

    drop_connect_rate = 0.2
    BN_MOMENTUM = 0.01

    bn_frozen = False

    def freeze_batchnorm(self, mode=True):
        self.bn_frozen = bool(mode)
        return self

    def forward(self, grd, sat, drop_masks=None):
        if self.training and self.precision != "fp32":
            raise NotImplementedError("ccvpe_amd: train mode is fp32 only")
        if not (grd.is_cuda and sat.is_cuda):
            raise RuntimeError("ccvpe_amd runs on the MI355X only: inputs must be device tensors")
        if self.training:
            from . import train
            if torch.is_grad_enabled() and any(p.requires_grad for p in self.parameters()):
                outs = train.apply(self, grd, sat, drop_masks)
            else:
                with torch.no_grad():
                    outs, _ = train.forward_train(self, grd, sat, drop_masks, rec=False)
            outs = list(outs)
            if self.ori_noise is not None:
                outs[3] = outs[3][:, len(self._loc_shifts()):]
            return tuple(outs)
        main = torch.cuda.current_stream()
        return self._forward_eval(grd, sat, main, self._side_stream() if EVAL_TWO_STREAMS else main)

    def _forward_eval(self, grd, sat, main, side):
        spec = MODEL_SPECS[self.kind]
        n_rot = spec["n_rot"]
        strides = MATCH_STRIDES[self.kind]
        circular = bool(self.circular_padding) and self.kind == "vigor"
        with torch.no_grad():
            pk = self._packed()
            grd = grd.contiguous().float()
            sat = sat.contiguous().float()
            batch = grd.shape[0]

            side.wait_stream(main)
            with torch.cuda.stream(side):
                gfeat, _ = _run_encoder(pk.grd, grd, circular, False, pk.dtype)
                _, gh, gw, _ = gfeat.shape
                if gh != spec["grd_h"]:
                    raise ValueError("ground feature height %d != %d expected by the descriptor heads"
                                     % (gh, spec["grd_h"]))
                y1 = _pw(gfeat, 1280, pk.gd_w, pk.gd_w3, pk.gd_n, batch=batch, in_h=gh, in_w=gw,
                         shift=pk.gd_bias, ldd=_round_up(pk.gd_n, 4), out_f32=True)
                gdesc = ops.ground_descriptor(y1, pk.gd_wh, pk.gd_bh, spec["cd"])
            svol, sfeats = _run_encoder(pk.sat, sat, False, True, pk.dtype)
            main.wait_stream(side)
            gdesc.record_stream(main)
            sdesc = _pw(svol, 1280, pk.sd_w, pk.sd_w3, pk.sd_n, batch=batch, in_h=svol.shape[1],
                        in_w=svol.shape[2], two=True, shift=pk.sd_bias)

            overlap = _overlap_decoders(self.precision, batch)
            loc_shifts = self._loc_shifts()
            fused = None
            scores_out = []
            smx = None
            x = sdesc
            cat6 = None
            goff = 0
            sfeats_loc = sfeats
            for j in range(6):
                lv = pk.loc[j]
                if j == pk.f32_from:
                    x = ops.cast_f32(x)
                    sfeats_loc = dict((SKIP_BLOCKS[q], ops.cast_f32(sfeats[SKIP_BLOCKS[q]])) for q in range(j, 5))
                hw = x.shape[1]
                cd = spec["cd"][j]
                L = gw * cd
                g = gdesc[:, goff:goff + L]
                goff += L
                if j == 0:
                    if self.ori_noise is None:
                        shifts, n_max = list(range(n_rot)), n_rot
                    else:
                        shifts, n_max = loc_shifts + list(range(n_rot)), len(loc_shifts)
                    n_tail = n_rot
                else:
                    shifts, n_max, n_tail = loc_shifts, len(loc_shifts), 0
                if fused is not None:
                    sc, cat = fused
                    fused = None
                else:
                    sc, cat = ops.match_level(x, g, L, shifts, n_max, n_tail, strides[j], lv.ldo, channels=lv.c,
                                              window_offset=window_offset(self.kind, lv.c, L))
                if j == 0:
                    cat6 = cat
                    scores_out.append(sc if self.ori_noise is None else sc[:, n_max:])
                    if overlap:
                        side.wait_stream(main)
                        with torch.cuda.stream(side):
                            x_ori = self._ori_decoder(pk, cat6, sfeats, batch)
                else:
                    scores_out.append(sc)
                skip = sfeats_loc[SKIP_BLOCKS[j]] if j < 5 else None
                if j == 5 and FUSE_TAIL and j in FOLD_LEVELS and ops.tail512_ok(hw, hw, lv.n_a):
                    logits_map, smx = ops.tail512(cat, lv.ldo, lv.fw, lv.fshift, lv.w_b, lv.b_b, 1, False, batch=batch, h1=hw, w1=hw,
                                                  split=_tail_split(self.precision, cat, 1),
                                                  want_softmax=True)
                    break
                if j in FOLD_LEVELS and batch * hw * hw >= FOLD_MIN_PIXELS:
                    y = _upconv_a(lv, cat, lv.ldo, batch, hw, skip)
                else:
                    up = ops.conv_igemm(cat, lv.ldo, lv.up_w, lv.up_n, batch=batch, in_h=hw, in_w=hw,
                                        shift=lv.up_b, out_mode=ops.OUT_DECONV2X, algo_k=lv.c + 1)
                    y = _double_conv(lv, up, skip, batch, 2 * hw)
                if j < 5:
                    to_f32 = j + 1 == pk.f32_from and y.dtype != torch.float32
                    nxt = pk.loc[j + 1]
                    L_n = gw * spec["cd"][j + 1]
                    if (FUSE_MATCH and len(loc_shifts) == 1 and
                            ops.conv3x3_match1(y, lv.n_a, lv.w_b, lv.n_b, None, L_n, loc_shifts[0], strides[j + 1], nxt.ldo, batch=batch,
                                               in_h=2 * hw, in_w=2 * hw, bias=lv.b_b, out_f32=to_f32, query_only=True)):
                        fused = ops.conv3x3_match1(y, lv.n_a, lv.w_b, lv.n_b, gdesc[:, goff:goff + L_n], L_n, loc_shifts[0],
                                                   strides[j + 1], nxt.ldo, batch=batch, in_h=2 * hw, in_w=2 * hw, bias=lv.b_b,
                                                   window_offset=window_offset(self.kind, nxt.c, L_n), out_f32=to_f32)
                        x = fused[1]
                    else:
                        x = _conv_b(lv, y, batch, 2 * hw, out_f32=to_f32)
                else:
                    logits_map = ops.head_conv3x3(y, lv.w_b, lv.b_b, 1, False)
            logits = logits_map.reshape(batch, -1)
            if smx is not None:
                heatmap = ops.softmax_apply(logits, smx).reshape(logits_map.shape)
            else:
                heatmap = ops.softmax_rows(logits).reshape(logits_map.shape)

            if overlap:
                main.wait_stream(side)
                x_ori.record_stream(main)
            else:
                x_ori = self._ori_decoder(pk, cat6, sfeats, batch)
        return (logits, heatmap, x_ori) + tuple(scores_out)


class CVM_VIGOR(_CVMBase):
    kind = "vigor"

    def __init__(self, device, circular_padding, efficientnet_weights=None):
        super().__init__(device, circular_padding, None, efficientnet_weights)


class CVM_VIGOR_ori_prior(_CVMBase):
    kind = "vigor"

    def __init__(self, device, ori_noise, circular_padding=True, efficientnet_weights=None):
        super().__init__(device, circular_padding, ori_noise, efficientnet_weights)


class CVM_OxfordRobotCar(_CVMBase):
    kind = "oxford"

    def __init__(self, device, efficientnet_weights=None):
        super().__init__(device, False, None, efficientnet_weights)


class CVM_KITTI(_CVMBase):
    kind = "kitti"

    def __init__(self, device, efficientnet_weights=None):
        super().__init__(device, False, None, efficientnet_weights)
```

ccvpe_amd/ops.py:

```python
import ctypes

import torch

from . import _lib
from ._lib import ConvDesc, check

ACT_NONE, ACT_RELU, ACT_SWISH, ACT_RELU_MASK = 0, 1, 2, 3
SPLIT_K_CALLS = 0
SPLIT_K = __import__("os").environ.get("CCVPE_SPLIT_K", "1") == "1"
OUT_NHWC, OUT_DECONV2X = 0, 1

_recorder = None


def set_recorder(rec):
    global _recorder
    _recorder = rec


class LaunchRecorder(object):

    def __init__(self):
        self.items = []

# ... 88 lines not shown
    return "%s_f32_kernel<%d,%d,%d>" % (fam, mt, nt, wn)


_record = None


def _empty(shape, device=None, dtype=torch.float32):
    if _record is not None:
        return _record.empty(shape, dtype, device)
    return torch.empty(shape, device=device, dtype=dtype)


def _ptr(t):
    if t is None:
        return None
    if _record is not None:
        _record.note(t)
    return ctypes.c_void_p(t.data_ptr())


def _chk(t, name, dtype=torch.float32):
    if t is None:
        return
    if not t.is_cuda or t.dtype != dtype or not t.is_contiguous():
        raise ValueError("%s must be a contiguous %s device tensor (got %s %s contiguous=%s)" % (
            name, dtype, t.device, t.dtype, t.is_contiguous()))


def _act_dtype(t):
    if t.dtype not in (torch.float32, torch.bfloat16):
        raise ValueError("activations must be fp32 or bf16, got %s" % t.dtype)
    return t.dtype


def conv_igemm(src0, c0, w_packed, n, *, batch, in_h, in_w, kh=1, kw=1, stride=1, pad=0,
               src1=None, c1=0, gate=None, scale=None, shift=None, residual=None, act=ACT_NONE,
               out_mode=OUT_NHWC, dst=None, ldd=None, ld0=None, ld1=None, algo_k=None, out_f32=False, route_only=False,
               variant_only=False):
    lib = _lib.load()
    dt = _act_dtype(src0)
    odt = torch.float32 if (out_f32 or dt == torch.float32) else dt
    for t, nm in ((src0, "src0"), (src1, "src1"), (w_packed, "w"), (residual, "residual")):
        _chk(t, nm, dt)
    for t, nm in ((gate, "gate"), (scale, "scale"), (shift, "shift")):
        _chk(t, nm)
    _chk(dst, "dst", odt)
    ld0 = ld0 if ld0 is not None else src0.shape[-1]
    ld1 = ld1 if ld1 is not None else (src1.shape[-1] if src1 is not None else 0)
    ho = (in_h + 2 * pad - kh) // stride + 1
    wo = (in_w + 2 * pad - kw) // stride + 1
    if out_mode == OUT_DECONV2X:
        cout = n // 4
        oshape = (batch, 2 * ho, 2 * wo)
    else:
        cout = n
        oshape = (batch, ho, wo)
    if dst is None:
        ldd = ldd if ldd is not None else cout
        dst = _empty(oshape + (ldd,), device=src0.device, dtype=odt)
    elif ldd is None:
        ldd = dst.shape[-1]
    d = ConvDesc()
    d.src0, d.src1, d.gate, d.w = _ptr(src0), _ptr(src1), _ptr(gate), _ptr(w_packed)
    d.scale, d.shift, d.residual, d.dst = _ptr(scale), _ptr(shift), _ptr(residual), _ptr(dst)
    d.c0, d.ld0, d.c1, d.ld1 = c0, ld0, c1, ld1
    d.batch, d.in_h, d.in_w = batch, in_h, in_w
    d.kh, d.kw, d.stride, d.pad = kh, kw, stride, pad
    d.n, d.kpad = n, w_packed.shape[1]
    d.ldd = ldd
    d.ldres = residual.shape[-1] if residual is not None else 0
    d.act, d.out_mode = act, out_mode
    if route_only:
        return conv_route(d, dt != torch.float32, bool(out_f32))
    if variant_only:
        return conv3x3_variant(d, dt != torch.float32)
    rec = _recorder
    ev0 = rec.begin() if rec is not None else None
    want = lib.ccvpe_conv_igemm_splitk_floats(ctypes.byref(d), int(dt != torch.float32)) if SPLIT_K else 0
    if want < 0:
        check(int(want), "ccvpe_conv_igemm_splitk_floats")
    if want > 0:
        global SPLIT_K_CALLS
        SPLIT_K_CALLS += 1
        scratch = _empty((want,), device=src0.device, dtype=torch.float32)
        if dt == torch.float32:
            check(lib.ccvpe_conv_igemm_splitk_f32(ctypes.byref(d), _ptr(scratch), _stream()), "ccvpe_conv_igemm_splitk_f32")
        else:
            check(lib.ccvpe_conv_igemm_splitk_bf16(ctypes.byref(d), int(bool(out_f32)), _ptr(scratch), _stream()),
                  "ccvpe_conv_igemm_splitk_bf16")
    elif dt == torch.float32:
        check(lib.ccvpe_conv_igemm_f32(ctypes.byref(d), _stream()), "ccvpe_conv_igemm_f32")
    else:
        check(lib.ccvpe_conv_igemm_bf16(ctypes.byref(d), int(bool(out_f32)), _stream()), "ccvpe_conv_igemm_bf16")
    if rec is not None:
        m = batch * ho * wo
        k_alg = algo_k if algo_k is not None else kh * kw * (c0 + c1)
        flops = 2.0 * m * n * k_alg
        esz = 4.0 if dt == torch.float32 else 2.0
        nbytes = esz * (batch * in_h * in_w * (c0 + c1) + m * n + n * k_alg
                        + (m * n if residual is not None else 0))
        if want > 0:
            name = igemm_tile(n, False)
        else:
            name = conv_route_name(d, dt != torch.float32, bool(out_f32))
        if want > 0 and dt != torch.float32:
            name = name.replace("_f32_kernel<", "_kernel<bf16,")
        rec.end(name, "%dx%d s%d M%d N%d K%d" % (kh, kw, stride, m, n, k_alg), flops, nbytes, ev0)
    return dst


def _wino_desc(src0, c0, u_packed, n, batch, in_h, in_w, shift, dst, ldd, ld0):
    d = ConvDesc()
    d.src0, d.src1, d.gate, d.w = _ptr(src0), None, None, _ptr(u_packed)
    d.scale, d.shift, d.residual, d.dst = None, _ptr(shift), None, _ptr(dst) if dst is not None else None
    d.c0, d.ld0, d.c1, d.ld1 = c0, ld0, 0, 0
    d.batch, d.in_h, d.in_w = batch, in_h, in_w
    d.kh, d.kw, d.stride, d.pad = 3, 3, 1, 1
    d.n, d.kpad = n, u_packed.shape[1]
    d.ldd, d.ldres = ldd, 0
    d.act, d.out_mode = ACT_NONE, OUT_NHWC
    return d


def conv3x3_wino_ok(src0, c0, u_packed, n, *, batch, in_h, in_w, ldd=None, ld0=None):
    if src0.dtype != torch.float32 or u_packed is None:
        return False
    ld0 = ld0 if ld0 is not None else src0.shape[-1]
    d = _wino_desc(src0, c0, u_packed, n, batch, in_h, in_w, None, None, ldd if ldd is not None else n, ld0)
    return bool(_lib.load().ccvpe_conv3x3_wino_ok(ctypes.byref(d)))


def conv3x3_wino(src0, c0, u_packed, n, *, batch, in_h, in_w, shift=None, dst=None, ldd=None, ld0=None):
    lib = _lib.load()
    for t, nm in ((src0, "src0"), (u_packed, "w"), (shift, "shift"), (dst, "dst")):
        _chk(t, nm)
    ld0 = ld0 if ld0 is not None else src0.shape[-1]
    if dst is None:
        ldd = ldd if ldd is not None else n
        dst = _empty((batch, in_h, in_w, ldd), device=src0.device)
    elif ldd is None:
        ldd = dst.shape[-1]
    d = _wino_desc(src0, c0, u_packed, n, batch, in_h, in_w, shift, dst, ldd, ld0)
    rec = _recorder
    ev0 = rec.begin() if rec is not None else None
    check(lib.ccvpe_conv3x3_wino_f32(ctypes.byref(d), _stream()), "ccvpe_conv3x3_wino_f32")
    if rec is not None:
        m = batch * in_h * in_w
        flops = 2.0 * m * n * 9 * c0
        nbytes = 4.0 * (m * c0 + m * n + n * 9 * c0)
        rec.end("conv3x3_wino_f32_kernel<16x16,32>", "3x3 s1 M%d N%d K%d" % (m, n, 9 * c0), flops, nbytes, ev0)
    return dst


def upconv3x3(src0, c0, w_packed, shift9, n, *, batch, h1, w1, src1=None, c1=0, act=ACT_NONE, algo_flops=None, route_only=False):
    lib = _lib.load()
    dt = _act_dtype(src0)
    for t, nm in ((src0, "src0"), (src1, "src1"), (w_packed, "w")):
        _chk(t, nm, dt)
    _chk(shift9, "shift9")
    dst = _empty((batch, 2 * h1, 2 * w1, n), device=src0.device, dtype=dt)
    d = _lib.UpconvDesc()
    d.src0, d.src1, d.w, d.shift9, d.dst = _ptr(src0), _ptr(src1), _ptr(w_packed), _ptr(shift9), _ptr(dst)
    d.c0, d.ld0, d.c1, d.ld1 = c0, src0.shape[-1], c1, (src1.shape[-1] if src1 is not None else 0)
    d.batch, d.h1, d.w1 = batch, h1, w1
    d.n, d.kpad, d.ldd, d.act = n, w_packed.shape[-1], n, act
    if route_only:
        return upconv_route(d, dt != torch.float32)
    rec = _recorder
    ev0 = rec.begin() if rec is not None else None
    fn = lib.ccvpe_upconv3x3_f32 if dt == torch.float32 else lib.ccvpe_upconv3x3_bf16
    check(fn(ctypes.byref(d), _stream()), "ccvpe_upconv3x3")
    if rec is not None:
        m = batch * h1 * w1 * 4
        k_eff = 4 * c0 + 9 * c1
        flops = algo_flops if algo_flops is not None else 2.0 * m * n * k_eff
        esz = 4.0 if dt == torch.float32 else 2.0
        nbytes = esz * (batch * h1 * w1 * c0 + m * c1 + m * n + 4 * n * k_eff)
        name = upconv_route_name(d, dt != torch.float32)
        rec.end(name, "up3x3 M%d N%d Keff%d" % (m, n, k_eff), flops, nbytes, ev0)
    return dst


def _s3_desc(src0, c0, w3_packed, shift9, n, batch, h1, w1, src1, c1, act, dst, ldd, ld0, ld1):
    d = _lib.UpconvDesc()
    d.src0, d.src1, d.w, d.shift9 = _ptr(src0), _ptr(src1), _ptr(w3_packed), _ptr(shift9)
    d.dst = _ptr(dst) if dst is not None else None
    d.c0, d.ld0, d.c1, d.ld1 = c0, ld0, c1, ld1
    d.batch, d.h1, d.w1 = batch, h1, w1
    d.n, d.kpad, d.ldd, d.act = n, w3_packed.shape[1] * w3_packed.shape[3], ldd, act
    return d


def upconv3x3_s3_ok(src0, c0, w3_packed, n, *, batch, h1, w1, src1=None, c1=0, ldd=None, ld0=None, ld1=None):
    if w3_packed is None or src0.dtype != torch.float32 or (src1 is not None and src1.dtype != torch.float32):
        return 0
    if w3_packed.dtype != torch.bfloat16 or w3_packed.dim() != 4:
        return 0
    ld0 = ld0 if ld0 is not None else src0.shape[-1]
    ld1 = ld1 if ld1 is not None else (src1.shape[-1] if src1 is not None else 0)
    d = _s3_desc(src0, c0, w3_packed, None, n, batch, h1, w1, src1, c1, ACT_NONE, None, ldd if ldd is not None else n, ld0, ld1)
    return int(_lib.load().ccvpe_upconv3x3_s3_ok(ctypes.byref(d)))


def upconv3x3_s3_form_ok(src0, c0, w3_packed, n, form, *, batch, h1, w1, src1=None, c1=0, ldd=None, ld0=None, ld1=None):
    if not upconv3x3_s3_ok(src0, c0, w3_packed, n, batch=batch, h1=h1, w1=w1, src1=src1, c1=c1, ldd=ldd, ld0=ld0, ld1=ld1):
        return 0
    ld0 = ld0 if ld0 is not None else src0.shape[-1]
    ld1 = ld1 if ld1 is not None else (src1.shape[-1] if src1 is not None else 0)
    d = _s3_desc(src0, c0, w3_packed, None, n, batch, h1, w1, src1, c1, ACT_NONE, None, ldd if ldd is not None else n, ld0, ld1)
    return int(_lib.load().ccvpe_upconv3x3_s3_form_ok(ctypes.byref(d), form))


def upconv3x3_s3(src0, c0, w3_packed, shift9, n, *, batch, h1, w1, src1=None, c1=0, act=ACT_NONE, dst=None, ldd=None, ld0=None,
                 ld1=None, form=None):
    lib = _lib.load()
    for t, nm in ((src0, "src0"), (src1, "src1"), (shift9, "shift9"), (dst, "dst")):
        _chk(t, nm)
    _chk(w3_packed, "w", torch.bfloat16)
    ld0 = ld0 if ld0 is not None else src0.shape[-1]
    ld1 = ld1 if ld1 is not None else (src1.shape[-1] if src1 is not None else 0)
    if dst is None:
        ldd = ldd if ldd is not None else n
        dst = _empty((batch, 2 * h1, 2 * w1, ldd), device=src0.device)
    elif ldd is None:
        ldd = dst.shape[-1]
    d = _s3_desc(src0, c0, w3_packed, shift9, n, batch, h1, w1, src1, c1, act, dst, ldd, ld0, ld1)
    rec = _recorder
    ev0 = rec.begin() if rec is not None else None
    if form is None:
        check(lib.ccvpe_upconv3x3_s3_f32(ctypes.byref(d), _stream()), "ccvpe_upconv3x3_s3_f32")
    else:
        check(lib.ccvpe_upconv3x3_s3_form_f32(ctypes.byref(d), form, _stream()), "ccvpe_upconv3x3_s3_form_f32")
    if rec is not None:
        m = batch * h1 * w1 * 4
        k_eff = 4 * c0 + 9 * c1
        flops = 2.0 * m * n * k_eff
        nbytes = 4.0 * (batch * h1 * w1 * c0 + m * c1 + m * n + 4 * n * k_eff)
        rec.end(upconv_s3_route_name(d, form or 0), "up3x3 M%d N%d Keff%d" % (m, n, k_eff), flops, nbytes, ev0)
    return dst


def _pw_s3_desc(src0, c0, w3_packed, n, batch, in_h, in_w, two, gate, scale, shift, residual, act, dst, ldd, ld0):
    d = ConvDesc()
    d.src0, d.src1, d.gate, d.w = _ptr(src0), None, _ptr(gate), _ptr(w3_packed)
    d.scale, d.shift, d.residual = _ptr(scale), _ptr(shift), _ptr(residual)
    d.dst = _ptr(dst) if dst is not None else None
    d.c0, d.ld0, d.c1, d.ld1 = c0, ld0, 0, 0
    d.batch, d.in_h, d.in_w = batch, in_h, in_w
    d.kh, d.kw, d.stride, d.pad = (2, 2, 2, 0) if two else (1, 1, 1, 0)
    d.n, d.kpad = n, w3_packed.shape[0] * w3_packed.shape[2]
    d.ldd = ldd
    d.ldres = residual.shape[-1] if residual is not None else 0
    d.act, d.out_mode = act, OUT_NHWC
    return d


def pw_s3_ok(src0, c0, w3_packed, n, *, batch, in_h, in_w, two=False, gate=None, residual=None, act=ACT_NONE, ldd=None, ld0=None):
    if w3_packed is None or src0.dtype != torch.float32 or (residual is not None and residual.dtype != torch.float32):
        return 0
    if w3_packed.dtype != torch.bfloat16 or w3_packed.dim() != 3 or w3_packed.shape[1] != (n + 15) // 16 * 16 or w3_packed.shape[2] != 48:
        return 0
    ld0 = ld0 if ld0 is not None else src0.shape[-1]
    d = _pw_s3_desc(src0, c0, w3_packed, n, batch, in_h, in_w, two, gate, None, None, residual, act, None, ldd if ldd is not None else n, ld0)
    return int(_lib.load().ccvpe_pw_s3_ok(ctypes.byref(d)))


def pw_s3_route_name(desc):
    r = _lib.load().ccvpe_pw_s3_route(ctypes.byref(desc))
    if r <= 0:
        raise _lib.CcvpeError("ccvpe_pw_s3_route: the kernel does not compute this layer")
    return "pw_s3_kernel<%d,%d,%d,%d>" % ((r >> 8) & 0xf, (r >> 12) & 0xf, (r >> 16) & 0xf, (r >> 20) & 0xf)


def pw_s3(src0, c0, w3_packed, n, *, batch, in_h, in_w, two=False, gate=None, scale=None, shift=None, residual=None, act=ACT_NONE,
          dst=None, ldd=None, ld0=None):
    lib = _lib.load()
    for t, nm in ((src0, "src0"), (gate, "gate"), (scale, "scale"), (shift, "shift"), (residual, "residual"), (dst, "dst")):
        _chk(t, nm)
    _chk(w3_packed, "w", torch.bfloat16)
    if w3_packed.dim() != 3 or w3_packed.shape[1] != (n + 15) // 16 * 16 or w3_packed.shape[2] != 48:
        raise ValueError("w is not the three-plane pack of models._pack_pw_s3 for n = %d" % n)
    ld0 = ld0 if ld0 is not None else src0.shape[-1]
    ho, wo = (in_h // 2, in_w // 2) if two else (in_h, in_w)
    if dst is None:
        ldd = ldd if ldd is not None else n
        dst = _empty((batch, ho, wo, ldd), device=src0.device)
    elif ldd is None:
        ldd = dst.shape[-1]
    d = _pw_s3_desc(src0, c0, w3_packed, n, batch, in_h, in_w, two, gate, scale, shift, residual, act, dst, ldd, ld0)
    rec = _recorder
    ev0 = rec.begin() if rec is not None else None
    check(lib.ccvpe_pw_s3_f32(ctypes.byref(d), _stream()), "ccvpe_pw_s3_f32")
    if rec is not None:
        m = batch * ho * wo
        k_alg = (4 if two else 1) * c0
        flops = 2.0 * m * n * k_alg
        nbytes = 4.0 * (batch * in_h * in_w * c0 + m * n + n * k_alg + (m * n if residual is not None else 0))
        rec.end(pw_s3_route_name(d), "%s M%d N%d K%d" % ("2x2 s2" if two else "1x1 s1", m, n, k_alg), flops, nbytes, ev0)
    return dst


def tail512(x, c0, w_packed, shift9, w2, b2, cout, normalize, *, batch, h1, w1, split=False, want_softmax=False):
    lib = _lib.load()
    dt = _act_dtype(x)
    _chk(x, "x", dt)
    _chk(w_packed, "w", dt)
# ... 65 lines not shown
    lib = _lib.load()
    for t, nm in ((x_nchw, "x"), (w, "w"), (s0, "s0"), (b0, "b0"), (w_dw, "w_dw"), (s1, "s1"), (b1, "b1")):
        _chk(t, nm)
    b, c, h, wd = x_nchw.shape
    if c != 3 or w_dw.numel() != 9 * 32:
        raise ValueError("stem_dw expects 3 input channels and a 3x3x32 depthwise weight")
    nblk = stem_dw_supported(h, wd, circular)
    if nblk <= 0:
        raise _lib.CcvpeError("stem_dw: unsupported shape %s" % (tuple(x_nchw.shape),))
    ho, wo = (h + 1 - 3) // 2 + 1, (wd + 1 - 3) // 2 + 1
    y = _empty((b, ho, wo, 32), device=x_nchw.device, dtype=out_dtype)
    part = _empty((b, nblk, 32), device=x_nchw.device, dtype=torch.float32)
    rec = _recorder
    ev0 = rec.begin() if rec is not None else None
    fn = lib.ccvpe_stem_dw_f32 if out_dtype == torch.float32 else lib.ccvpe_stem_dw_bf16
    check(fn(_ptr(x_nchw), _ptr(w), _ptr(s0), _ptr(b0), _ptr(w_dw), _ptr(s1), _ptr(b1), _ptr(y), _ptr(part), b, h, wd,
             int(bool(circular)), _stream()), "ccvpe_stem_dw")
    if rec is not None:
        flops = 2.0 * b * ho * wo * 32 * (27 + 9)
        nbytes = 4.0 * b * 3 * h * wd + (4.0 if out_dtype == torch.float32 else 2.0) * b * ho * wo * 32
        rec.end("stem_dw_kernel", "in %dx%dx3" % (h, wd), flops, nbytes, ev0)
    return y, part


def dwconv(x, w, scale, shift, k, stride, circular):
    lib = _lib.load()
    dt = _act_dtype(x)
    _chk(x, "x", dt)
    for t, nm in ((w, "w"), (scale, "scale"), (shift, "shift")):
        _chk(t, nm)
    b, h, wd, c = x.shape
    tot = (k - 1) if stride == 1 else (k - 2)
    ho, wo = (h + tot - k) // stride + 1, (wd + tot - k) // stride + 1
    nblk = lib.ccvpe_dwconv_nblk(h, wd, c, stride)
    if nblk <= 0:
        raise _lib.CcvpeError("ccvpe_dwconv_nblk rejected shape %s" % (tuple(x.shape),))
    y = _empty((b, ho, wo, c), device=x.device, dtype=dt)
    part = _empty((b, nblk, c), device=x.device, dtype=torch.float32)
    fn = lib.ccvpe_dwconv_f32 if dt == torch.float32 else lib.ccvpe_dwconv_bf16
    check(fn(_ptr(x), _ptr(w), _ptr(scale), _ptr(shift), _ptr(y), _ptr(part), b, h, wd, c, k, stride,
             int(bool(circular)), _stream()), "ccvpe_dwconv")
    return y, part


def mbconv_front_supported(in_h, in_w, cin, mid, k, stride):
    n = _lib.load().ccvpe_mbconv_front_nblk(in_h, in_w, cin, mid, k, stride)
    if n < 0:
        raise _lib.CcvpeError("ccvpe_mbconv_front_nblk rejected k=%d stride=%d" % (k, stride))
    return n


def mbconv_band_plan(in_h, in_w, cin, mid, k, stride, batch):
    r = _lib.load().ccvpe_mbconv_band_plan(in_h, in_w, cin, mid, k, stride, batch)
    if r <= 0:
        return None
    return dict(nkk=r & 0xf, tpw=(r >> 4) & 0xf, ry=(r >> 8) & 0xf, cpg=(r >> 12) & 0xff, ngrp=(r >> 20) & 0xff)


def mbconv_front(x, w_exp, s0, b0, w_dw, s1, b1, mid, k, stride, circular):
    lib = _lib.load()
    dt = _act_dtype(x)
    _chk(x, "x", dt)
    _chk(w_exp, "w_exp", dt)
    for t, nm in ((s0, "s0"), (b0, "b0"), (w_dw, "w_dw"), (s1, "s1"), (b1, "b1")):
        _chk(t, nm)
    b, h, wd, cin = x.shape
    nblk = mbconv_front_supported(h, wd, cin, mid, k, stride)
    if nblk == 0:
        raise _lib.CcvpeError("mbconv_front: unsupported shape %s" % (tuple(x.shape),))
    tot = (k - 1) if stride == 1 else (k - 2)
    ho, wo = (h + tot - k) // stride + 1, (wd + tot - k) // stride + 1
    y = _empty((b, ho, wo, mid), device=x.device, dtype=dt)
    part = _empty((b, nblk, mid), device=x.device, dtype=torch.float32)
    rec = _recorder
    ev0 = rec.begin() if rec is not None else None
    fn = lib.ccvpe_mbconv_front_f32 if dt == torch.float32 else lib.ccvpe_mbconv_front_bf16
    check(fn(_ptr(x), _ptr(w_exp), w_exp.shape[1], _ptr(s0), _ptr(b0), _ptr(w_dw), _ptr(s1), _ptr(b1), _ptr(y),
             _ptr(part), b, h, wd, cin, mid, k, stride, int(bool(circular)), _stream()), "ccvpe_mbconv_front")
    if rec is not None:
        flops = 2.0 * b * h * wd * cin * mid + 2.0 * b * ho * wo * mid * k * k
        nbytes = (4.0 if dt == torch.float32 else 2.0) * (b * h * wd * cin + b * ho * wo * mid)
        route = lib.ccvpe_mbconv_front_route(h, wd, cin, mid, k, stride, int(dt != torch.float32), b)
        kname = {1: "mbconv_front_kernel", 2: "mbconv_plane_kernel", 3: "mbconv_band_kernel"}.get(route, "mbconv_front_kernel")
        rec.end("%s<%d,%d>" % (kname, k, stride), "in %dx%dx%d mid %d" % (h, wd, cin, mid), flops, nbytes, ev0)
    return y, part


def mbconv_front_s3_ok(x, w_exp3, mid, k, stride):
    if w_exp3 is None or x.dtype != torch.float32 or w_exp3.dtype != torch.bfloat16:
        return 0
    b, h, wd, cin = x.shape
    if w_exp3.dim() != 3 or tuple(w_exp3.shape) != ((cin + 15) // 16, mid, 48):
        return 0
    return int(_lib.load().ccvpe_mbconv_front_s3_ok(h, wd, cin, mid, k, stride, b))


def mbconv_front_s3(x, w_exp3, s0, b0, w_dw, s1, b1, mid, k, stride, circular):
    lib = _lib.load()
    _chk(x, "x", torch.float32)
    _chk(w_exp3, "w_exp3", torch.bfloat16)
    for t, nm in ((s0, "s0"), (b0, "b0"), (w_dw, "w_dw"), (s1, "s1"), (b1, "b1")):
        _chk(t, nm)
    b, h, wd, cin = x.shape
    if w_exp3.dim() != 3 or tuple(w_exp3.shape) != ((cin + 15) // 16, mid, 48):
        raise ValueError("w_exp3 is not the three-plane pack of models._pack_pw_s3 for cin = %d, mid = %d" % (cin, mid))
    nblk = mbconv_front_supported(h, wd, cin, mid, k, stride)
    if nblk == 0 or not lib.ccvpe_mbconv_front_s3_ok(h, wd, cin, mid, k, stride, b):
        raise _lib.CcvpeError("mbconv_front_s3: unsupported shape %s k=%d stride=%d" % (tuple(x.shape), k, stride))
    tot = (k - 1) if stride == 1 else (k - 2)
    ho, wo = (h + tot - k) // stride + 1, (wd + tot - k) // stride + 1
    y = _empty((b, ho, wo, mid), device=x.device, dtype=torch.float32)
    part = _empty((b, nblk, mid), device=x.device, dtype=torch.float32)
    rec = _recorder
    ev0 = rec.begin() if rec is not None else None
    check(lib.ccvpe_mbconv_front_s3_f32(_ptr(x), _ptr(w_exp3), w_exp3.shape[0] * w_exp3.shape[2], _ptr(s0), _ptr(b0), _ptr(w_dw),
                                        _ptr(s1), _ptr(b1), _ptr(y), _ptr(part), b, h, wd, cin, mid, k, stride,
                                        int(bool(circular)), _stream()), "ccvpe_mbconv_front_s3_f32")
    if rec is not None:
        flops = 2.0 * b * h * wd * cin * mid + 2.0 * b * ho * wo * mid * k * k
        nbytes = 4.0 * (b * h * wd * cin + b * ho * wo * mid)
        rec.end("mbconv_front_s3_kernel<%d,%d>" % (k, stride), "in %dx%dx%d mid %d" % (h, wd, cin, mid), flops, nbytes, ev0)
    return y, part


def se_gate(part, hw, w1, b1, w2, b2):
    lib = _lib.load()
    for t, nm in ((part, "part"), (w1, "w1"), (b1, "b1"), (w2, "w2"), (b2, "b2")):
        _chk(t, nm)
    b, nblk, c = part.shape
    cs = w1.shape[0]
    gate = _empty((b, c), device=part.device, dtype=torch.float32)
    check(lib.ccvpe_se_gate_f32(_ptr(part), nblk, 1.0 / float(hw), _ptr(w1), _ptr(b1), _ptr(w2), _ptr(b2),
                                _ptr(gate), b, c, cs, _stream()), "ccvpe_se_gate_f32")
    return gate


def ground_descriptor(y1, wh, bh, cd):
    lib = _lib.load()
    for t, nm in ((y1, "y1"), (wh, "wh"), (bh, "bh")):
        _chk(t, nm)
    b, h, w, ld = y1.shape
    cd_arr = (ctypes.c_int * 6)(*cd)
    out = _empty((b, w * sum(cd)), device=y1.device, dtype=torch.float32)
    check(lib.ccvpe_ground_descriptor_f32(_ptr(y1), ld, _ptr(wh), _ptr(bh), cd_arr, _ptr(out), b, h, w,
                                          _stream()), "ccvpe_ground_descriptor_f32")
    return out


def conv3x3_match1(src0, c0, w_packed, n, g, L, shift, stride, ldo, *, batch, in_h, in_w, bias, window_offset=0, out_f32=False,
                   query_only=False):
    lib = _lib.load()
    dt = _act_dtype(src0)
    if dt != torch.bfloat16:
        if query_only:
            return False
        raise ValueError("conv3x3_match1: bf16 storage only")
    _chk(src0, "src0", dt)
    _chk(w_packed, "w", dt)
    _chk(bias, "bias")
    d = ConvDesc()
    d.src0, d.src1, d.gate, d.w = _ptr(src0), None, None, _ptr(w_packed)
    d.scale, d.shift, d.residual = None, _ptr(bias), None
    d.c0, d.ld0, d.c1, d.ld1 = c0, src0.shape[-1], 0, 0
    d.batch, d.in_h, d.in_w = batch, in_h, in_w
    d.kh, d.kw, d.stride, d.pad = 3, 3, 1, 1
    d.n, d.kpad, d.ldd, d.ldres = n, w_packed.shape[1], ldo, 0
    d.act, d.out_mode = ACT_NONE, OUT_NHWC
    if query_only:
        return lib.ccvpe_conv3x3_match1_ok(ctypes.byref(d), int(bool(out_f32)), L) == 1
    if not g.is_cuda or g.dtype != torch.float32 or g.stride(-1) != 1:
        raise ValueError("g must be an fp32 device tensor with unit inner stride")
    scores = _empty((batch, 1, in_h, in_w), device=src0.device, dtype=torch.float32)
    cat = _empty((batch, in_h, in_w, ldo), device=src0.device, dtype=torch.float32 if out_f32 else dt)
    d.dst = _ptr(cat)
    rec = _recorder
    ev0 = rec.begin() if rec is not None else None
    check(lib.ccvpe_conv3x3_match1_bf16(ctypes.byref(d), int(bool(out_f32)), _ptr(g), g.stride(0), L, int(shift), int(stride),
                                        int(window_offset), _ptr(scores), _stream()), "ccvpe_conv3x3_match1_bf16")
    if rec is not None:
        m = batch * in_h * in_w
        rec.end("c3n_kernel<bf16,%d,match>" % n, "3x3+match M%d N%d K%d" % (m, n, 9 * c0), 2.0 * m * n * 9 * c0,
                2.0 * m * c0 + (4.0 if out_f32 else 2.0) * m * ldo + 4.0 * m + 2.0 * n * 9 * c0, ev0)
    return scores, cat


def match_level(x, g, L, shifts, n_max, n_tail, stride, ldo, channels=None, window_offset=0):
    lib = _lib.load()
    dt = _act_dtype(x)
    _chk(x, "x", dt)
    if not g.is_cuda or g.dtype != torch.float32 or g.stride(-1) != 1:
        raise ValueError("g must be an fp32 device tensor with unit inner stride")
    b, h, w, ldx = x.shape
    c = channels if channels is not None else ldx
    n = len(shifts)
    sh = (ctypes.c_int * n)(*shifts)
    scores = _empty((b, n, h, w), device=x.device, dtype=torch.float32)
    dstx = _empty((b, h, w, ldo), device=x.device, dtype=dt)
    fn = lib.ccvpe_match_level_f32 if dt == torch.float32 else lib.ccvpe_match_level_bf16
    check(fn(_ptr(x), ldx, _ptr(g), g.stride(0), L, sh, n, n_max, n_tail, stride, window_offset, _ptr(scores), _ptr(dstx),
             ldo, b, h * w, c, _stream()), "ccvpe_match_level")
    return scores, dstx


def head_conv3x3(x, w, bias, cout, normalize):
    lib = _lib.load()
    dt = _act_dtype(x)
    _chk(x, "x", dt)
    for t, nm in ((w, "w"), (bias, "bias")):
        _chk(t, nm)
    b, h, wd, c = x.shape
    if c != 16:
        raise ValueError("head conv expects 16 input channels")
    out = _empty((b, cout, h, wd), device=x.device, dtype=torch.float32)
    fn = lib.ccvpe_head_conv3x3_f32 if dt == torch.float32 else lib.ccvpe_head_conv3x3_bf16
    check(fn(_ptr(x), _ptr(w), _ptr(bias), _ptr(out), b, h, wd, cout, int(bool(normalize)), _stream()),
          "ccvpe_head_conv3x3")
    return out


def cast_f32(x):
    if x.dtype == torch.float32:
        return x
    lib = _lib.load()
    _chk(x, "x", torch.bfloat16)
    out = _empty(x.shape, device=x.device, dtype=torch.float32)
    check(lib.ccvpe_cast_bf16_f32(_ptr(x), _ptr(out), x.numel(), _stream()), "ccvpe_cast_bf16_f32")
    return out


def softmax_rows(logits):
    lib = _lib.load()
    _chk(logits, "logits")
    rows, n = logits.shape
    out = _empty(logits.shape, device=logits.device, dtype=logits.dtype)
    check(lib.ccvpe_softmax_rows_f32(_ptr(logits), _ptr(out), rows, n, _stream()), "ccvpe_softmax_rows_f32")
    return out


def stem_conv_raw(x_nchw, w, circular):
    lib = _lib.load()
    _chk(x_nchw, "x")
    _chk(w, "w")
    b, c, h, wd = x_nchw.shape
    ho, wo = (h + 1 - 3) // 2 + 1, (wd + 1 - 3) // 2 + 1
    y = _empty((b, ho, wo, 32), device=x_nchw.device, dtype=torch.float32)
    check(lib.ccvpe_stem_conv_raw_f32(_ptr(x_nchw), _ptr(w), _ptr(y), b, h, wd, int(bool(circular)), _stream()),
          "ccvpe_stem_conv_raw_f32")
    return y


def dwconv_raw(x, w, k, stride, circular):
    lib = _lib.load()
    _chk(x, "x")
    _chk(w, "w")
    b, h, wd, c = x.shape
    tot = (k - 1) if stride == 1 else (k - 2)
    ho, wo = (h + tot - k) // stride + 1, (wd + tot - k) // stride + 1
    y = _empty((b, ho, wo, c), device=x.device, dtype=torch.float32)
    check(lib.ccvpe_dwconv_raw_f32(_ptr(x), _ptr(w), _ptr(y), b, h, wd, c, k, stride, int(bool(circular)), _stream()),
          "ccvpe_dwconv_raw_f32")
    return y


def bn_stats(x, run_mean=None, run_var=None, momentum=0.01):
    lib = _lib.load()
    _chk(x, "x")
    _chk(run_mean, "run_mean")
    _chk(run_var, "run_var")
    c = x.shape[-1]
    rows = x.numel() // c
    mean = _empty((c,), device=x.device, dtype=torch.float32)
    var = _empty((c,), device=x.device, dtype=torch.float32)
    scratch = _empty((lib.ccvpe_bn_stats_nblk(rows) * 3 * c,), device=x.device, dtype=torch.float32)
    check(lib.ccvpe_bn_stats_f32(_ptr(x), rows, c, _ptr(mean), _ptr(var), _ptr(run_mean), _ptr(run_var),
                                 float(momentum), _ptr(scratch), _stream()), "ccvpe_bn_stats_f32")
    return mean, var


def bn_act(x, mean, var, gamma, beta, eps, act, residual=None, dc_scale=None, want_se=False):
    lib = _lib.load()
    for t, nm in ((x, "x"), (mean, "mean"), (var, "var"), (gamma, "gamma"), (beta, "beta"), (residual, "residual"),
                  (dc_scale, "dc_scale")):
        _chk(t, nm)
    b, c = x.shape[0], x.shape[-1]
    rps = x.numel() // (b * c)
    y = _empty(x.shape, device=x.device, dtype=x.dtype)
    part = None
    if want_se:
        part = _empty((b, lib.ccvpe_bn_act_nblk(rps), c), device=x.device, dtype=torch.float32)
    check(lib.ccvpe_bn_act_f32(_ptr(x), _ptr(mean), _ptr(var), _ptr(gamma), _ptr(beta), float(eps), act, _ptr(residual),
                               _ptr(dc_scale), _ptr(y), _ptr(part), b, rps, c, _stream()), "ccvpe_bn_act_f32")
    return (y, part) if want_se else y


def eval_postprocess(heatmap, ori):
    lib = _lib.load()
    _chk(heatmap, "heatmap")
    _chk(ori, "ori")
    b, _, h, w = heatmap.shape
    out = _empty((b, 6), device=heatmap.device, dtype=torch.float32)
    check(lib.ccvpe_eval_postprocess_f32(_ptr(heatmap), _ptr(ori), _ptr(out), b, h, w, _stream()),
          "ccvpe_eval_postprocess_f32")
    return out


def eval_metrics(heatmap, ori, gt, gt_ori, heading_deg, metres_per_pixel, out=None):
    lib = _lib.load()
    for t, nm in ((heatmap, "heatmap"), (ori, "ori"), (gt, "gt"), (gt_ori, "gt_ori")):
        _chk(t, nm)
# ... 107 lines not shown
```

ccvpe_amd/plan.py:

```python
import ctypes
import struct
import weakref

import torch

from . import _lib, ops

K_INT, K_FLT, K_NULL, K_WEIGHTS, K_WORKSPACE, K_GRD, K_SAT, K_STREAM, K_BLOB = range(9)
ALIGN = 256

LAUNCHES = ("ccvpe_conv_igemm_f32", "ccvpe_conv_igemm_bf16", "ccvpe_conv_igemm_splitk_f32", "ccvpe_conv_igemm_splitk_bf16",
            "ccvpe_conv3x3_match1_bf16", "ccvpe_conv3x3_wino_f32",
            "ccvpe_upconv3x3_f32", "ccvpe_upconv3x3_bf16", "ccvpe_upconv3x3_s3_f32", "ccvpe_pw_s3_f32", "ccvpe_tail512_f32", "ccvpe_tail512_bf16", "ccvpe_stem_conv_f32",
            "ccvpe_stem_conv_bf16", "ccvpe_stem_dw_f32", "ccvpe_stem_dw_bf16", "ccvpe_dwconv_f32", "ccvpe_dwconv_bf16", "ccvpe_mbconv_front_f32", "ccvpe_mbconv_front_bf16", "ccvpe_mbconv_front_s3_f32",
            "ccvpe_se_gate_f32", "ccvpe_ground_descriptor_f32", "ccvpe_match_level_f32", "ccvpe_match_level_bf16",
            "ccvpe_head_conv3x3_f32", "ccvpe_head_conv3x3_bf16", "ccvpe_softmax_rows_f32", "ccvpe_softmax_apply_f32", "ccvpe_cast_bf16_f32",
            "ccvpe_eval_postprocess_f32")
QUERIES = ("ccvpe_tail512_partials", "ccvpe_conv3x3_match1_ok", "ccvpe_conv3x3_wino_ok", "ccvpe_upconv3x3_s3_ok", "ccvpe_conv_igemm_splitk_floats", "ccvpe_conv_igemm_route", "ccvpe_conv3x3_variant", "ccvpe_upconv3x3_route", "ccvpe_upconv3x3_s3_route", "ccvpe_pw_s3_ok", "ccvpe_pw_s3_route", "ccvpe_dwconv_nblk", "ccvpe_mbconv_front_nblk", "ccvpe_mbconv_front_route", "ccvpe_mbconv_front_s3_ok", "ccvpe_mbconv_band_plan", "ccvpe_stem_dw_nblk",
           "ccvpe_last_error", "ccvpe_abi_version")


class _Arena(object):

    def __init__(self, size):
        self.size, self.free, self.peak = size, [(0, size)], 0

    def alloc(self, nbytes):
        n = max(ALIGN, (nbytes + ALIGN - 1) // ALIGN * ALIGN)
        for i, (off, sz) in enumerate(self.free):
            if sz >= n:
                if sz == n:
                    del self.free[i]
                else:
                    self.free[i] = (off + n, sz - n)
                self.peak = max(self.peak, off + n)
                return off, n
        raise MemoryError("plan arena exhausted")

    def release(self, off, n):
        fr = self.free
        lo, hi = 0, len(fr)
        while lo < hi:
            mid = (lo + hi) // 2
            if fr[mid][0] < off:
                lo = mid + 1
            else:
                hi = mid
        fr.insert(lo, (off, n))
        if lo + 1 < len(fr) and fr[lo][0] + fr[lo][1] == fr[lo + 1][0]:
            fr[lo] = (fr[lo][0], fr[lo][1] + fr[lo + 1][1])
            del fr[lo + 1]
        if lo > 0 and fr[lo - 1][0] + fr[lo - 1][1] == fr[lo][0]:
            fr[lo - 1] = (fr[lo - 1][0], fr[lo - 1][1] + fr[lo][1])
            del fr[lo]


def _tensor_ranges(obj, out=None, seen=None):
    out = [] if out is None else out
    seen = set() if seen is None else seen
    if id(obj) in seen:
        return out
    seen.add(id(obj))
    if isinstance(obj, torch.Tensor):
        if obj.is_cuda and obj.numel():
            st = obj.untyped_storage()
            out.append((st.data_ptr(), st.data_ptr() + st.nbytes()))
    elif isinstance(obj, dict):
        for v in obj.values():
            _tensor_ranges(v, out, seen)
    elif isinstance(obj, (list, tuple)):
        for v in obj:
            _tensor_ranges(v, out, seen)
    elif hasattr(obj, "__dict__"):
        _tensor_ranges(vars(obj), out, seen)
    return out


class _Recorder(object):
    def __init__(self, device, arena_bytes, grd, sat, side_fraction=0.45, constants=None):
        self.ws = torch.empty((arena_bytes,), dtype=torch.uint8, device=device)
        self.base = self.ws.data_ptr()
        self.split = int(arena_bytes * (1.0 - side_fraction)) // ALIGN * ALIGN
        self.arenas = (_Arena(self.split), _Arena(arena_bytes - self.split))
        self.size = arena_bytes
        self.grd, self.sat = grd, sat
        self.calls, self.blobs = [], []
        self.weights, self.weights_bytes = {}, 0
        self.seen = {}
        self.constants = sorted(constants) if constants is not None else None
        self.main = torch.cuda.current_stream().cuda_stream
        self.quarantine = []
        self.n_waits = 0

    def sid(self):
        return 0 if torch.cuda.current_stream().cuda_stream == self.main else 1

    @property
    def peak(self):
        return max(self.arenas[0].peak, self.split + self.arenas[1].peak if self.arenas[1].peak else 0)

    def empty(self, shape, dtype, device):
        shape = tuple(int(s) for s in shape)
        n = 1
        for s in shape:
            n *= s
        item = torch.empty((), dtype=dtype).element_size()
        region = self.sid()
        off, size = self.arenas[region].alloc(n * item)
        goff = off + (self.split if region else 0)
        t = torch.empty((0,), dtype=dtype, device=device).set_(self.ws.untyped_storage(), goff // item, shape)
        weakref.finalize(t, self._release, region, off, size)
        return t

    def _release(self, region, off, size):
        if self.sid() == region:
            self.arenas[region].release(off, size)
        else:
            self.quarantine.append((region, off, size))

    def wait(self, waiter, waitee):
        a = 0 if waiter.cuda_stream == self.main else 1
        b = 0 if waitee.cuda_stream == self.main else 1
        if a == b:
            return
        self.calls.append(("@wait", [(K_INT, a), (K_INT, b)], a))
        self.n_waits += 1
        if a == 0:
            for region, off, size in self.quarantine:
                self.arenas[region].release(off, size)
            self.quarantine = []

    def note(self, t):
        p = t.data_ptr()
        if not (self.base <= p < self.base + self.size):
            self._check_constant(p, t.numel() * t.element_size())
            self.seen[p] = t

    def _is_input(self, addr):
        for t in (self.grd, self.sat):
            p = t.data_ptr()
            if p <= addr < p + t.numel() * t.element_size():
                return True
        return False

    def _check_constant(self, addr, nbytes=1):
        if self.constants is None or self._is_input(addr):
            return
        import bisect
        i = bisect.bisect_right(self.constants, (addr, float("inf"))) - 1
        if i >= 0 and self.constants[i][0] <= addr and addr + max(nbytes, 1) <= self.constants[i][1]:
            return
        raise RuntimeError("plan: pointer 0x%x (%d bytes) is neither workspace, nor an input, nor part of the weights packed before "
                           "recording: an intermediate allocated outside ops._empty would be frozen as a constant" % (addr, nbytes))

    def classify(self, addr):
        if addr is None or addr == 0:
            return K_NULL, 0
        if self.base <= addr < self.base + self.size:
            return K_WORKSPACE, addr - self.base
        for kind, t in ((K_GRD, self.grd), (K_SAT, self.sat)):
            p = t.data_ptr()
            if p <= addr < p + t.numel() * t.element_size():
                return kind, addr - p
        return K_WEIGHTS, self._weight_offset(addr)

    def _weight_offset(self, addr):
        self._check_constant(addr)
        if addr in self.weights:
            return self.weights[addr][0]
        t = self.seen.get(addr)
        if t is None:
# ... 200 lines not shown
```

include/ccvpe_hip.h:

```cpp
#ifndef CCVPE_HIP_H
#define CCVPE_HIP_H

#ifdef __cplusplus
extern "C" {
#endif

#define CCVPE_OK 0
#define CCVPE_EINVAL (-1)
#define CCVPE_ELAUNCH (-2)

#define CCVPE_ACT_NONE 0
#define CCVPE_ACT_RELU 1
#define CCVPE_ACT_SWISH 2
#define CCVPE_ACT_RELU_MASK 3

#define CCVPE_OUT_NHWC 0
#define CCVPE_OUT_DECONV2X 1

#define CCVPE_MAX_SHIFTS 48

const char* ccvpe_last_error(void);
int ccvpe_abi_version(void);

typedef struct ccvpe_conv_desc {
  const float* src0;
  const float* src1;
  const float* gate;
  const float* w;
  const float* scale;
  const float* shift;
  const float* residual;
  float* dst;
  int c0, ld0, c1, ld1;
  int batch, in_h, in_w;
  int kh, kw, stride, pad;
  int n;
  int kpad;
  int ldd, ldres;
  int act;
  int out_mode;
} ccvpe_conv_desc;

int ccvpe_conv_igemm_f32(const ccvpe_conv_desc* desc, void* stream);

int ccvpe_conv_igemm_splitk_floats(const ccvpe_conv_desc* desc, int is_bf16);
#define CCVPE_ROUTE_IGEMM 0
#define CCVPE_ROUTE_PW_GEMM 1
#define CCVPE_ROUTE_CONV3X3 2
#define CCVPE_ROUTE_C3N 3
#define CCVPE_ROUTE_PW_RING 4
#define CCVPE_ROUTE_PWN 5
int ccvpe_conv_igemm_route(const ccvpe_conv_desc* desc, int is_bf16, int out_f32);
int ccvpe_conv3x3_variant(const ccvpe_conv_desc* desc, int is_bf16);
int ccvpe_set_narrow_kernels(int on);
int ccvpe_set_pw_ring_kernels(int on);
int ccvpe_set_pwn_kernels(int on);
int ccvpe_set_mbconv_plane_kernels(int mode);
int ccvpe_conv3x3_wino_ok(const ccvpe_conv_desc* desc);
int ccvpe_conv3x3_wino_f32(const ccvpe_conv_desc* desc, void* stream);
int ccvpe_conv3x3_match1_ok(const ccvpe_conv_desc* desc, int out_f32, int L);
int ccvpe_conv3x3_match1_bf16(const ccvpe_conv_desc* desc, int out_f32, const float* g, int ldg, int L, int shift, int stride,
                              int window_offset, float* scores, void* stream);
int ccvpe_conv_igemm_splitk_f32(const ccvpe_conv_desc* desc, float* scratch, void* stream);

typedef struct ccvpe_upconv_desc {
  const void* src0;
  const void* src1;
  const void* w;
  const float* shift9;
  void* dst;
  int c0, ld0, c1, ld1;
  int batch, h1, w1;
  int n, kpad, ldd;
  int act;
} ccvpe_upconv_desc;

int ccvpe_upconv3x3_f32(const ccvpe_upconv_desc* desc, void* stream);
int ccvpe_upconv3x3_bf16(const ccvpe_upconv_desc* desc, void* stream);
#define CCVPE_UPROUTE_GATHER 0
#define CCVPE_UPROUTE_HALO 1
#define CCVPE_UPROUTE_DMA 2
#define CCVPE_UPROUTE_DMA_PAIR 3
#define CCVPE_UPROUTE_UP2 4
int ccvpe_upconv3x3_route(const ccvpe_upconv_desc* desc, int is_bf16);
int ccvpe_upconv3x3_s3_ok(const ccvpe_upconv_desc* desc);
int ccvpe_upconv3x3_s3_f32(const ccvpe_upconv_desc* desc, void* stream);
int ccvpe_upconv3x3_s3_form_ok(const ccvpe_upconv_desc* desc, int form);
int ccvpe_upconv3x3_s3_route(const ccvpe_upconv_desc* desc, int form);
int ccvpe_upconv3x3_s3_form_f32(const ccvpe_upconv_desc* desc, int form, void* stream);
int ccvpe_set_s3_quad(int on);
int ccvpe_pw_s3_ok(const ccvpe_conv_desc* desc);
int ccvpe_pw_s3_route(const ccvpe_conv_desc* desc);
int ccvpe_pw_s3_f32(const ccvpe_conv_desc* desc, void* stream);

typedef struct ccvpe_tail_desc {
  const void* x;
  const void* w;
  const float* shift9;
  const float* w2;
  const float* b2;
  float* out;
  int batch, h1, w1;
  int c0, ld0, kpad;
  int cout, normalize, split;
  float* softmax_partial;
} ccvpe_tail_desc;

int ccvpe_tail512_f32(const ccvpe_tail_desc* desc, void* stream);
int ccvpe_tail512_bf16(const ccvpe_tail_desc* desc, void* stream);
int ccvpe_tail512_partials(const ccvpe_tail_desc* desc, int is_bf16);
int ccvpe_softmax_apply_f32(const float* logits, const float* partials, int n_partials, float* out, int rows, int n,
                            void* stream);

typedef struct ccvpe_ctx ccvpe_ctx;
int ccvpe_ctx_create(const void* plan, long long n_bytes, void* weights_dev, void* workspace_dev, ccvpe_ctx** ctx);
int ccvpe_ctx_destroy(ccvpe_ctx* ctx);
int ccvpe_ctx_info(const ccvpe_ctx* ctx, long long* workspace_bytes, long long* weights_bytes, long long* grd_bytes,
                   long long* sat_bytes, int* n_outputs, int* n_calls);
int ccvpe_ctx_output(const ccvpe_ctx* ctx, int i, void** dev_ptr, long long* bytes, int* ndim, long long* dims4,
                     long long* strides4);
int ccvpe_forward(ccvpe_ctx* ctx, const void* grd, const void* sat, void** out, void* stream);

int ccvpe_stem_conv_f32(const float* x_nchw, const float* w, const float* scale, const float* shift,
                        float* y, int batch, int in_h, int in_w, int circular, void* stream);

int ccvpe_dwconv_nblk(int in_h, int in_w, int channels, int stride);
int ccvpe_dwconv_f32(const float* x, const float* w, const float* scale, const float* shift, float* y,
                     float* se_partial, int batch, int in_h, int in_w, int channels, int k, int stride,
                     int circular, void* stream);

int ccvpe_stem_dw_nblk(int in_h, int in_w, int circular);
int ccvpe_stem_dw_f32(const float* x_nchw, const float* w, const float* s0, const float* b0, const float* w_dw,
                      const float* s1, const float* b1, float* y, float* se_partial, int batch, int in_h,
                      int in_w, int circular, void* stream);
int ccvpe_stem_dw_bf16(const float* x_nchw, const float* w, const float* s0, const float* b0, const float* w_dw,
                       const float* s1, const float* b1, void* y, float* se_partial, int batch, int in_h,
                       int in_w, int circular, void* stream);

int ccvpe_mbconv_front_nblk(int in_h, int in_w, int cin, int mid, int k, int stride);
int ccvpe_mbconv_front_route(int in_h, int in_w, int cin, int mid, int k, int stride, int is_bf16, int batch);
int ccvpe_mbconv_band_plan(int in_h, int in_w, int cin, int mid, int k, int stride, int batch);
int ccvpe_mbconv_front_f32(const float* x, const float* w_exp, int kpad, const float* s0, const float* b0,
                           const float* w_dw, const float* s1, const float* b1, float* y, float* se_partial,
                           int batch, int in_h, int in_w, int cin, int mid, int k, int stride, int circular,
                           void* stream);
int ccvpe_mbconv_front_s3_ok(int in_h, int in_w, int cin, int mid, int k, int stride, int batch);
int ccvpe_mbconv_front_s3_f32(const float* x, const void* w_exp3, int kpad, const float* s0, const float* b0,
                              const float* w_dw, const float* s1, const float* b1, float* y, float* se_partial,
                              int batch, int in_h, int in_w, int cin, int mid, int k, int stride, int circular,
                              void* stream);

int ccvpe_se_gate_f32(const float* se_partial, int nblk, float inv_hw, const float* w1, const float* b1,
                      const float* w2, const float* b2, float* gate, int batch, int channels,
                      int squeezed, void* stream);

int ccvpe_ground_descriptor_f32(const float* y1, int ld, const float* wh, const float* bh, const int* cd,
                                float* out, int batch, int h, int w, void* stream);

int ccvpe_set_match_mfma(int on);
#define CCVPE_MATCH_ROUTE_INTS 10
int ccvpe_match_route(int elem_size, int L, const int* shifts, int n_shifts, int n_max, int n_tail, int stride,
                      int window_offset, int ldx, int ldo, int batch, int hw, int channels, int* out);
int ccvpe_match_level_f32(const float* x, int ldx, const float* g, int ldg, int L, const int* shifts,
                          int n_shifts, int n_max, int n_tail, int stride, int window_offset, float* scores,
                          float* dstx, int ldo, int batch, int hw, int channels, void* stream);

int ccvpe_head_conv3x3_f32(const float* x, const float* w, const float* bias, float* out_nchw, int batch,
                           int h, int w_, int cout, int normalize, void* stream);

int ccvpe_softmax_rows_f32(const float* logits, float* out, int rows, int n, void* stream);
int ccvpe_multi_copy_f32(const void* const* srcs, void* const* dsts, const int* counts, int n, void* stream);
int ccvpe_gather_repack_f32(void* const* dsts, const void* const* srcs, const long long* idx_off, const int* counts,
                            const int* idx, int n_chunks, void* stream);
int ccvpe_gather_repack_chunk(void);
int ccvpe_cast_bf16_f32(const void* src, float* dst, long n_elems, void* stream);

int ccvpe_eval_postprocess_f32(const float* heatmap, const float* ori, float* out, int batch, int h, int w,
                               void* stream);

int ccvpe_eval_metrics_f32(const float* heatmap, const float* ori, const float* gt, const float* gt_ori,
                           const double* heading_deg, const double* metres_per_pixel, double* rows, int batch, int h,
                           int w, void* stream);

int ccvpe_belief_partials(int h, int w);
int ccvpe_belief_step_f32(const float* prior, const float* heat, const float* ori, const int* offsets, const float* taps,
                          int radius, float outlier, const int* reset, float* post, double* scratch, double* rows,
                          int batch, int h, int w, void* stream);

int ccvpe_infonce_scratch_floats(int batch, int n);
int ccvpe_infonce_loss_f32(const float* scores, const float* labels, float temperature, float* loss,
                           float* rows, float* scratch, int batch, int n, void* stream);
int ccvpe_cross_entropy_loss_f32(const float* logits, const float* labels, float* loss, float* scratch,
                                 int batch, int n, void* stream);
int ccvpe_orientation_loss_f32(const float* ori, const float* gt_ori, const float* gt, float* loss,
                               float* scratch, int batch, int hw, void* stream);

int ccvpe_stem_conv_raw_f32(const float* x_nchw, const float* w, float* y, int batch, int in_h, int in_w,
                            int circular, void* stream);
int ccvpe_dwconv_raw_f32(const float* x, const float* w, float* y, int batch, int in_h, int in_w, int channels,
                         int k, int stride, int circular, void* stream);
int ccvpe_bn_stats_nblk(int rows);
int ccvpe_bn_stats_f32(const float* x, int rows, int channels, float* mean, float* var, float* run_mean,
                       float* run_var, float momentum, float* scratch, void* stream);
int ccvpe_bn_act_nblk(int rows_per_sample);
int ccvpe_bn_act_f32(const float* x, const float* mean, const float* var, const float* gamma, const float* beta,
                     float eps, int act, const float* residual, const float* dc_scale, float* y,
                     float* se_partial, int batch, int rows_per_sample, int channels, void* stream);

int ccvpe_conv_wgrad_tile(int n, int ncols);
int ccvpe_conv_wgrad_scratch_floats(int batch, int in_h, int in_w, int kh, int kw, int stride, int pad, int ctot,
                                    int n);
int ccvpe_conv_wgrad_f32(const float* src0, int c0, int ld0, const float* src1, int c1, int ld1, const float* dy,
// ... 133 lines not shown
```

Before: 2868.

## Add narrow-N Winograd 3x3 kernel with fused fp32 match epilogue

Adds a new Winograd F(2x2,3x3) kernel for narrow output widths (17-80 channels). It splits the transform across wave pairs that exchange partial results through LDS, and offers an optional fused matching epilogue that computes per-pixel L2 normalisation and the cosine score against the ground descriptor. The model routes fp32 decoder 3x3 convs and the conv+match step onto it when the shape gate allows, replacing the direct implicit-GEMM path. The aim is to cut FLOPs and an extra pass over activations. In exchange it adds LDS exchange synchronisation and pixel-count heuristics for when to use it.

```diff
diff --git a/ccvpe_amd/_lib.py b/ccvpe_amd/_lib.py
--- a/ccvpe_amd/_lib.py
+++ b/ccvpe_amd/_lib.py
@@ -74,6 +74,11 @@
     "ccvpe_set_pwn_kernels": (c_int, [c_int]),
     "ccvpe_conv3x3_wino_ok": (c_int, [ctypes.POINTER(ConvDesc)]),
     "ccvpe_conv3x3_wino_f32": (c_int, [ctypes.POINTER(ConvDesc), c_void_p]),
+    "ccvpe_conv3x3_wino_n_ok": (c_int, [ctypes.POINTER(ConvDesc)]),
+    "ccvpe_conv3x3_wino_n_f32": (c_int, [ctypes.POINTER(ConvDesc), c_void_p]),
+    "ccvpe_conv3x3_wino_match1_ok": (c_int, [ctypes.POINTER(ConvDesc), c_int, c_int]),
+    "ccvpe_conv3x3_wino_match1_f32": (c_int, [ctypes.POINTER(ConvDesc), c_int, c_void_p, c_int, c_int, c_int, c_int, c_int, c_void_p, c_void_p]),
+    "ccvpe_set_wino_n": (c_int, [c_int]),
     "ccvpe_conv3x3_match1_ok": (c_int, [ctypes.POINTER(ConvDesc), c_int, c_int]),
     "ccvpe_conv3x3_match1_bf16": (c_int, [ctypes.POINTER(ConvDesc), c_int, c_void_p, c_int, c_int, c_int, c_int, c_int, c_void_p, c_void_p]),
     "ccvpe_conv_igemm_splitk_f32": (c_int, [ctypes.POINTER(ConvDesc), c_void_p, c_void_p]),
@@ -234,6 +239,8 @@
         lib.ccvpe_set_pwn_kernels(0)
     if os.environ.get("CCVPE_S3_QUAD") == "0" and hasattr(lib, "ccvpe_set_s3_quad"):
         lib.ccvpe_set_s3_quad(0)
+    if os.environ.get("CCVPE_WINO_N") == "0" and hasattr(lib, "ccvpe_set_wino_n"):
+        lib.ccvpe_set_wino_n(0)
     if os.environ.get("CCVPE_MBPLANE") is not None and hasattr(lib, "ccvpe_set_mbconv_plane_kernels"):
         lib.ccvpe_set_mbconv_plane_kernels(int(os.environ["CCVPE_MBPLANE"]))
     _lib = lib
diff --git a/ccvpe_amd/csrc/conv3x3_wino.hip b/ccvpe_amd/csrc/conv3x3_wino.hip
--- a/ccvpe_amd/csrc/conv3x3_wino.hip
+++ b/ccvpe_amd/csrc/conv3x3_wino.hip
@@ -209,7 +209,7 @@
 
 static int round_up(int v, int m) { return (v + m - 1) / m * m; }
 
-static const char* wino_refusal(const ccvpe_conv_desc* d) {
+const char* wino_shape_refusal(const ccvpe_conv_desc* d) {
   if (!d) return "null desc";
   if (d->kh != 3 || d->kw != 3 || d->stride != 1 || d->pad != 1 || d->out_mode != CCVPE_OUT_NHWC) return "3x3 / stride 1 / pad 1 / NHWC only";
   if (d->c1 != 0 || d->src1 || d->gate || d->scale || d->residual || d->act != CCVPE_ACT_NONE)
@@ -218,10 +218,16 @@
   if (d->c0 < 32 || d->c0 % 4 || d->ld0 < d->c0 || d->ld0 % 4) return "c0 >= 32, c0 and ld0 multiples of 4";
   if (d->n <= 0 || d->ldd < d->n || d->ldd % 4) return "ldd >= n, ldd multiple of 4";
   if (d->kpad != 16 * round_up(d->c0, 16)) return "kpad must be 16 * round_up(c0, 16) (packed U)";
-  if ((long)d->batch * d->in_h * d->in_w < 16384) return "fewer than 16384 output pixels";
+  if (d->batch <= 0) return "batch must be positive";
   if ((long)d->batch * d->in_h * d->in_w > 0x7fffffffL) return "too many pixels";
   if ((size_t)round_up(d->n, WG_BN) * d->kpad * 4 >= (1ull << 32)) return "U larger than 4 GB";
   if (!aligned16(d->src0) || !aligned16(d->w) || !aligned16(d->dst)) return "pointers must be 16-byte aligned";
+  return nullptr;
+}
+
+const char* wino_refusal(const ccvpe_conv_desc* d) {
+  if (const char* why = wino_shape_refusal(d)) return why;
+  if ((long)d->batch * d->in_h * d->in_w < 16384) return "fewer than 16384 output pixels";
   ccvpe_conv_desc dd = *d;
   dd.kpad = round_up(9 * d->c0, 16);
   if (ccvpe_conv_igemm_splitk_floats(&dd, 0) != 0) return "the direct path splits K at this shape";
@@ -235,7 +241,7 @@
 extern "C" int ccvpe_conv3x3_wino_ok(const ccvpe_conv_desc* d) { return wino_refusal(d) ? 0 : 1; }
 
 extern "C" int ccvpe_conv3x3_wino_f32(const ccvpe_conv_desc* d, void* stream) {
-  if (const char* why = wino_refusal(d)) return fail(CCVPE_EINVAL, "conv3x3_wino: %s", why);
+  if (const char* why = wino_shape_refusal(d)) return fail(CCVPE_EINVAL, "conv3x3_wino: %s", why);
   IgemmParams p{};
   p.src0 = d->src0; p.w = d->w; p.shift = d->shift; p.dst = d->dst;
   p.c0 = d->c0; p.ld0 = d->ld0;
diff --git a/ccvpe_amd/csrc/conv3x3_wino_n.hip b/ccvpe_amd/csrc/conv3x3_wino_n.hip
--- /dev/null
+++ b/ccvpe_amd/csrc/conv3x3_wino_n.hip
@@ -0,0 +1,450 @@
+#include "conv_common.h"
+
+namespace ccvpe {
+
+struct WinoNParams {
+  const float* src0;
+  const float* w;
+  const float* shift;
+  float* dst;
+  int c0, ld0, H, W, N, Kpad, ldd;
+  int tiles_x, tiles_y, tiles_total;
+  const float* g;
+  float* scores;
+  int ldg, L, off;
+};
+
+static constexpr int WN_HC = 18;
+static constexpr int WN_TAB = 176;
+static constexpr int WN_XCH = 8 * 64 * 4;
+constexpr int wn_halo_floats(int ns) { return (4 * ns + 2) * WN_HC * LDS_LD; }
+constexpr int wn_lds_bytes(int nt, int ns) {
+  const int work = wn_halo_floats(ns) + 2 * 8 * 16 * nt * 16, xch = 2 * ns * WN_XCH;
+  return (WN_TAB + (work > xch ? work : xch)) * 4;
+}
+
+template <int NT, bool MATCH, int NS>
+__global__ __launch_bounds__(128 * NS, 2) void conv3x3_wino_n_kernel(const WinoNParams p) {
+  constexpr int WN_NW = 2 * NS;
+  constexpr int WN_HPX = (4 * NS + 2) * WN_HC;
+  constexpr int WN_HS = wn_halo_floats(NS);
+  constexpr int NTHR = 64 * WN_NW;
+  constexpr int NPAD = 16 * NT;
+  constexpr int H_IT = (WN_HPX * 4 + NTHR - 1) / NTHR;
+  constexpr int NP = (NT + 1) / 2;
+  extern __shared__ __attribute__((aligned(16))) float wn_sm[];
+  float* mtab = wn_sm;
+  float* Hs = wn_sm + WN_TAB;
+  float* Bs = Hs + WN_HS;
+  float* Xs = Hs;
+
+  const int tid = threadIdx.x;
+  const int lane = tid & 63;
+  const int wave = sgpr(tid >> 6);
+  const int strip = wave % NS, G = wave / NS;
+
+  const int tile = xcd_tile(blockIdx.x, p.tiles_total);
+  const int tx = tile % p.tiles_x;
+  const int ty = (tile / p.tiles_x) % p.tiles_y;
+  const int b = tile / (p.tiles_x * p.tiles_y);
+  const int y0 = ty * (4 * NS), x0 = tx * 16;
+  const int ctot = p.c0;
+  const int cpad = p.Kpad / 16;
+  const int nchunks = (ctot + 15) / 16;
+  const int nstages = nchunks * 2;
+  const float* src0 = p.src0;
+  const float* wp = p.w;
+
+  int h_off[H_IT], h_pix[H_IT], h_sub[H_IT];
+#pragma unroll
+  for (int it = 0; it < H_IT; ++it) {
+    const int idx = tid + NTHR * it;
+    const int px = idx >> 2, sub = idx & 3;
+    h_sub[it] = sub;
+    if (px < WN_HPX) {
+      const int hy = px / WN_HC, hx = px - hy * WN_HC;
+      const int iy = y0 - 1 + hy, ix = x0 - 1 + hx;
+      h_off[it] = px * LDS_LD + sub * 4;
+      h_pix[it] = ((unsigned)iy < (unsigned)p.H && (unsigned)ix < (unsigned)p.W) ? (b * p.H + iy) * p.W + ix : -1;
+    } else {
+      h_off[it] = -1;
+      h_pix[it] = -1;
+    }
+  }
+  f32x4 h_reg[H_IT];
+  int h_chunk = 0;
+  const int ld0s = sgpr(p.ld0);
+  auto load_halo = [&](int chunk) {
+    h_chunk = chunk;
+#pragma unroll
+    for (int it = 0; it < H_IT; ++it) {
+      const int ch = chunk * 16 + h_sub[it] * 4;
+      const bool ok = h_pix[it] >= 0 && ch < ctot;
+      const size_t off = ok ? (size_t)h_pix[it] * ld0s + ch : 0;
+      h_reg[it] = *reinterpret_cast<const f32x4*>(src0 + off);
+    }
+  };
+  auto store_halo = [&]() {
+#pragma unroll
+    for (int it = 0; it < H_IT; ++it)
+      if (h_off[it] >= 0)
+        *reinterpret_cast<f32x4*>(Hs + h_off[it]) = keep_if(h_reg[it], h_pix[it] >= 0 && h_chunk * 16 + h_sub[it] * 4 < ctot);
+  };
+
+  const int rl = lane >> 2;
+  const unsigned wvoff = ((unsigned)rl * (unsigned)p.Kpad + (unsigned)(((lane & 3) ^ w_swz(rl)) * 4)) * 4u;
+  const unsigned bs_lds = (unsigned)(uintptr_t)(__attribute__((address_space(3))) float*)Bs;
+  auto load_w = [&](int chunk, int r, int dbuf) {
+#pragma unroll
+    for (int i = 0; i < 8 / WN_NW; ++i) {
+      const int slot = wave + i * WN_NW;
+      const int comp = ((slot >> 2) * 2 + r) * 4 + (slot & 3);
+#pragma unroll
+      for (int q = 0; q < NT; ++q) {
+        const char* sbase = reinterpret_cast<const char*>(wp) + ((size_t)comp * cpad + (size_t)chunk * 16 + (size_t)q * 16 * p.Kpad) * 4;
+        const unsigned lds = __builtin_amdgcn_readfirstlane(bs_lds + (unsigned)(((dbuf * 8 + slot) * NPAD + q * 16) * 16 * 4));
+        asm volatile("s_mov_b32 m0, %0\n\tglobal_load_lds_dwordx4 %1, %2" ::"s"(lds), "v"(wvoff), "s"(sbase) : "memory", "m0");
+      }
+    }
+  };
+  auto dma_wait = [&]() { asm volatile("s_waitcnt vmcnt(0)" ::: "memory"); };
+
+  f32x4 acc[2][4][NT];
+#pragma unroll
+  for (int r = 0; r < 2; ++r)
+#pragma unroll
+    for (int x = 0; x < 4; ++x)
+#pragma unroll
+      for (int j = 0; j < NT; ++j) acc[r][x][j] = (f32x4){0.f, 0.f, 0.f, 0.f};
+
+  const int frow = lane & 15;
+  const int fk = (lane >> 4) * 4;
+  const int bcol = ((lane >> 4) ^ w_swz(frow)) * 4;
+  const int ttx = frow & 7, tty = frow >> 3;
+  const int dbase = ((4 * strip + 2 * tty) * WN_HC + 2 * ttx) * LDS_LD + fk;
+  const int rowa0 = 2 * G * WN_HC * LDS_LD, rowb0 = (2 - G) * WN_HC * LDS_LD;
+  const int rowa1 = WN_HC * LDS_LD, rowb1 = (2 + G) * WN_HC * LDS_LD;
+
+  load_halo(0);
+  load_w(0, 0, 0);
+  if constexpr (MATCH) {
+    if (tid < NPAD) {
+      int k = tid + p.off;
+      k = k >= p.N ? k - p.N : k;
+      const bool in = tid < p.N && k < p.L;
+      mtab[tid] = in ? p.g[(size_t)b * p.ldg + k] : 0.f;
+      mtab[80 + tid] = in ? 1.f : 0.f;
+    }
+    if (wave == WN_NW - 1) {
+      const float v0 = lane < p.L ? p.g[(size_t)b * p.ldg + lane] : 0.f;
+      const float v1 = lane + 64 < p.L ? p.g[(size_t)b * p.ldg + lane + 64] : 0.f;
+      float s = fmaf(v1, v1, v0 * v0);
+#pragma unroll
+      for (int m = 32; m >= 1; m >>= 1) s += __shfl_xor(s, m, 64);
+      if (lane == 0) mtab[160] = sqrtf(s);
+    }
+  }
+  store_halo();
+  dma_wait();
+  __syncthreads();
+
+  int chunk = 0;
+  auto stage = [&](int s, auto rtag) {
+    constexpr int R = decltype(rtag)::value;
+    const bool more = s + 1 < nstages;
+    if (R == 0 && chunk + 1 < nchunks) load_halo(chunk + 1);
+    if (more) load_w(R == 1 ? chunk + 1 : chunk, R ^ 1, (s + 1) & 1);
+
+    f32x4 v[4];
+    {
+      f32x4 t[4];
+      const float* pa = Hs + dbase + (R == 0 ? rowa0 : rowa1);
+      const float* pb = Hs + dbase + (R == 0 ? rowb0 : rowb1);
+#pragma unroll
+      for (int x = 0; x < 4; ++x) {
+        const f32x4 da = *reinterpret_cast<const f32x4*>(pa + x * LDS_LD);
+        const f32x4 db = *reinterpret_cast<const f32x4*>(pb + x * LDS_LD);
+        if (R == 1 && G == 0) t[x] = da + db;
+        else t[x] = da - db;
+      }
+      v[0] = t[0] - t[2];
+      v[1] = t[1] + t[2];
+      v[2] = t[2] - t[1];
+      v[3] = t[1] - t[3];
+    }
+    __builtin_amdgcn_sched_barrier(0);
+#pragma unroll
+    for (int x = 0; x < 4; ++x) {
+      f32x4 bf[NT];
+#pragma unroll
+      for (int j = 0; j < NT; ++j)
+        bf[j] = *reinterpret_cast<const f32x4*>(&Bs[(((s & 1) * 8 + G * 4 + x) * NPAD + j * 16 + frow) * 16 + bcol]);
+#pragma unroll
+      for (int kk = 0; kk < 4; ++kk)
+#pragma unroll
+        for (int j = 0; j < NT; ++j)
+          acc[R][x][j] = __builtin_amdgcn_mfma_f32_16x16x4f32(bf[j][kk], v[x][kk], acc[R][x][j], 0, 0, 0);
+    }
+    __builtin_amdgcn_sched_barrier(0);
+    dma_wait();
+    __syncthreads();
+    if (R == 1 && more) {
+      store_halo();
+      __syncthreads();
+    }
+  };
+  for (int s = 0; s < nstages; s += 2, ++chunk) {
+    stage(s, std::integral_constant<int, 0>{});
+    stage(s + 1, std::integral_constant<int, 1>{});
+  }
+
+  const int oy = y0 + 4 * strip + 2 * tty, ox = x0 + 2 * ttx;
+  const bool inside = oy < p.H && ox < p.W;
+  const size_t m00 = (size_t)(b * p.H + oy) * p.W + ox;
+  f32x4* xmine = reinterpret_cast<f32x4*>(Xs + wave * WN_XCH) + lane;
+  const f32x4* xpeer = reinterpret_cast<const f32x4*>(Xs + (wave ^ NS) * WN_XCH) + lane;
+
+  f32x4 yk[MATCH ? NP : 1][2][2];
+  if constexpr (MATCH) {
+#pragma unroll
+    for (int q = 0; q < NP; ++q)
+#pragma unroll
+      for (int i = 0; i < 4; ++i) yk[q][i >> 1][i & 1] = (f32x4){0.f, 0.f, 0.f, 0.f};
+  }
+
+  auto send = [&](auto jtag) {
+    constexpr int J = decltype(jtag)::value;
+#pragma unroll
+    for (int r = 0; r < 2; ++r)
+#pragma unroll
+      for (int x = 0; x < 4; ++x) xmine[(r * 4 + x) * 64] = acc[r][x][J];
+  };
+  auto finish = [&](const f32x4 (&m)[4][4], int j, f32x4 (&y)[2][2]) {
+    const int n = j * 16 + fk;
+    f32x4 q0[4], q1[4];
+#pragma unroll
+    for (int c = 0; c < 4; ++c) {
+      q0[c] = m[0][c] + m[1][c] + m[2][c];
+      q1[c] = m[1][c] - m[2][c] - m[3][c];
+    }
+    f32x4 bias;
+#pragma unroll
+    for (int r = 0; r < 4; ++r) bias[r] = (p.shift && n + r < p.N) ? p.shift[n + r] : 0.0f;
+    y[0][0] = q0[0] + q0[1] + q0[2] + bias;
+    y[0][1] = q0[1] - q0[2] - q0[3] + bias;
+    y[1][0] = q1[0] + q1[1] + q1[2] + bias;
+    y[1][1] = q1[1] - q1[2] - q1[3] + bias;
+  };
+  auto store_block = [&](int j, const f32x4 (&y)[2][2]) {
+    const int n = j * 16 + fk;
+    if (!inside || n >= p.N) return;
+#pragma unroll
+    for (int dy = 0; dy < 2; ++dy)
+#pragma unroll
+      for (int dx = 0; dx < 2; ++dx) {
+        const size_t o = (m00 + (size_t)dy * p.W + dx) * p.ldd + n;
+        if (n + 3 < p.N) {
+          *reinterpret_cast<f32x4*>(p.dst + o) = y[dy][dx];
+        } else {
+#pragma unroll
+          for (int r = 0; r < 4; ++r)
+            if (n + r < p.N) p.dst[o + r] = y[dy][dx][r];
+        }
+      }
+  };
+  auto round = [&](auto ptag) {
+    constexpr int P = decltype(ptag)::value;
+    constexpr int JE = 2 * P, JO = 2 * P + 1;
+    if (G == 0) {
+      if constexpr (JO < NT) send(std::integral_constant<int, JO>{});
+    } else {
+      send(std::integral_constant<int, JE>{});
+    }
+    __syncthreads();
+    f32x4 y[2][2];
+    if (G == 0) {
+      f32x4 m[4][4];
+#pragma unroll
+      for (int x = 0; x < 4; ++x) {
+        m[0][x] = acc[0][x][JE];
+        m[1][x] = acc[1][x][JE];
+        m[2][x] = xpeer[x * 64];
+        m[3][x] = xpeer[(4 + x) * 64];
+      }
+      finish(m, JE, y);
+      if constexpr (!MATCH) store_block(JE, y);
+    } else if constexpr (JO < NT) {
+      f32x4 m[4][4];
+#pragma unroll
+      for (int x = 0; x < 4; ++x) {
+        m[0][x] = xpeer[x * 64];
+        m[1][x] = xpeer[(4 + x) * 64];
+        m[2][x] = acc[0][x][JO];
+        m[3][x] = acc[1][x][JO];
+      }
+      finish(m, JO, y);
+      if constexpr (!MATCH) store_block(JO, y);
+    }
+    if constexpr (MATCH) {
+      if (G == 0 || JO < NT) {
+#pragma unroll
+        for (int i = 0; i < 4; ++i) yk[P][i >> 1][i & 1] = y[i >> 1][i & 1];
+      }
+    }
+    __syncthreads();
+  };
+  round(std::integral_constant<int, 0>{});
+  if constexpr (NP > 1) round(std::integral_constant<int, 1>{});
+  if constexpr (NP > 2) round(std::integral_constant<int, 2>{});
+
+  if constexpr (MATCH) {
+    float s2[4], wn[4], dt[4];
+#pragma unroll
+    for (int i = 0; i < 4; ++i) s2[i] = wn[i] = dt[i] = 0.f;
+#pragma unroll
+    for (int q = 0; q < NP; ++q) {
+      const int n = (2 * q + G) * 16 + fk;
+      if (2 * q + G < NT) {
+        const f32x4 gq = *reinterpret_cast<const f32x4*>(mtab + n);
+        const f32x4 wq = *reinterpret_cast<const f32x4*>(mtab + 80 + n);
+#pragma unroll
+        for (int i = 0; i < 4; ++i)
+#pragma unroll
+          for (int r = 0; r < 4; ++r) {
+            const float x = yk[q][i >> 1][i & 1][r];
+            const float x2 = x * x;
+            s2[i] += x2;
+            wn[i] = fmaf(x2, wq[r], wn[i]);
+            dt[i] = fmaf(x, gq[r], dt[i]);
+          }
+      }
+    }
+#pragma unroll
+    for (int i = 0; i < 4; ++i) {
+      s2[i] += __shfl_xor(s2[i], 16, 64); wn[i] += __shfl_xor(wn[i], 16, 64); dt[i] += __shfl_xor(dt[i], 16, 64);
+      s2[i] += __shfl_xor(s2[i], 32, 64); wn[i] += __shfl_xor(wn[i], 32, 64); dt[i] += __shfl_xor(dt[i], 32, 64);
+    }
+    float* rmine = Xs + wave * WN_XCH + lane;
+    const float* rpeer = Xs + (wave ^ NS) * WN_XCH + lane;
+#pragma unroll
+    for (int i = 0; i < 4; ++i) {
+      rmine[(i * 3 + 0) * 64] = s2[i];
+      rmine[(i * 3 + 1) * 64] = wn[i];
+      rmine[(i * 3 + 2) * 64] = dt[i];
+    }
+    __syncthreads();
+    const float gnorm = mtab[160];
+    float inv[4], score[4];
+#pragma unroll
+    for (int i = 0; i < 4; ++i) {
+      const float a = rpeer[(i * 3 + 0) * 64], bw = rpeer[(i * 3 + 1) * 64], c = rpeer[(i * 3 + 2) * 64];
+      const float ts = G == 0 ? s2[i] + a : a + s2[i];
+      const float tw = G == 0 ? wn[i] + bw : bw + wn[i];
+      const float td = G == 0 ? dt[i] + c : c + dt[i];
+      inv[i] = 1.0f / fmaxf(sqrtf(ts), 1e-12f);
+      score[i] = td / (sqrtf(tw) * gnorm);
+    }
+#pragma unroll
+    for (int q = 0; q < NP; ++q) {
+      if (2 * q + G < NT) {
+        f32x4 y[2][2];
+#pragma unroll
+        for (int i = 0; i < 4; ++i) y[i >> 1][i & 1] = yk[q][i >> 1][i & 1] * inv[i];
+        store_block(2 * q + G, y);
+      }
+    }
+    if (G == 0 && inside) {
+#pragma unroll
+      for (int i = 0; i < 4; ++i) {
+        const size_t pix = m00 + (size_t)(i >> 1) * p.W + (i & 1);
+        for (int k = p.N + fk; k < p.ldd; k += 16)
+          *reinterpret_cast<f32x4*>(p.dst + pix * p.ldd + k) = (f32x4){k == p.N ? score[i] : 0.f, 0.f, 0.f, 0.f};
+        if (fk == 0) p.scores[pix] = score[i];
+      }
+    }
+  }
+}
+
+static int round_up_n(int v, int m) { return (v + m - 1) / m * m; }
+
+static bool g_wino_n = true;
+
+static long wino_n_min_pixels(int nt) { return nt >= 4 ? 1L << 17 : 1L << 19; }
+
+static int wino_n_level(const ccvpe_conv_desc* d, bool match) {
+  if (wino_shape_refusal(d)) return 0;
+  if (d->n <= 16 || d->n > 80) return 0;
+  if (match && (d->n % 4 || d->ldd < d->n + 1)) return 0;
+  if (!g_wino_n || wino_refusal(d)) return 1;
+  if (round_up_n(d->n, 16) == round_up_n(d->n, 32)) return 1;
+  return (long)d->batch * d->in_h * d->in_w >= wino_n_min_pixels(round_up_n(d->n, 16) / 16) ? 2 : 1;
+}
+
+template <bool MATCH>
+static int wino_n_run(const ccvpe_conv_desc* d, WinoNParams& p, hipStream_t stream) {
+  p.src0 = reinterpret_cast<const float*>(d->src0); p.w = reinterpret_cast<const float*>(d->w);
+  p.shift = d->shift; p.dst = reinterpret_cast<float*>(d->dst);
+  p.c0 = d->c0; p.ld0 = d->ld0;
+  p.H = d->in_h; p.W = d->in_w;
+  p.N = d->n; p.Kpad = d->kpad; p.ldd = d->ldd;
+  p.tiles_x = (p.W + 15) / 16;
+  const int nt = round_up_n(d->n, 16) / 16;
+  const int ns = nt == 3 ? 2 : 4;
+  p.tiles_y = (p.H + 4 * ns - 1) / (4 * ns);
+  const long total = (long)p.tiles_x * p.tiles_y * d->batch;
+  if (total > 0x7fffffffL) return fail(CCVPE_EINVAL, "conv3x3_wino_n: grid too large");
+  p.tiles_total = (int)total;
+  static DevCache lds_set[4];
+  void (*kern)(const WinoNParams) = nullptr;
+  switch (nt) {
+    case 2: kern = conv3x3_wino_n_kernel<2, MATCH, 4>; break;
+    case 3: kern = conv3x3_wino_n_kernel<3, MATCH, 2>; break;
+    case 4: kern = conv3x3_wino_n_kernel<4, MATCH, 4>; break;
+    case 5: kern = conv3x3_wino_n_kernel<5, MATCH, 4>; break;
+    default: return fail(CCVPE_EINVAL, "conv3x3_wino_n: 16 < n <= 80 only");
+  }
+  const int lds = wn_lds_bytes(nt, ns);
+  if (int rc = ensure_dyn_lds(lds_set[nt - 2], kern, lds, "conv3x3_wino_n")) return rc;
+  hipLaunchKernelGGL(kern, dim3(p.tiles_total), dim3(128 * ns), lds, stream, p);
+  return check_launch(MATCH ? "conv3x3_wino_n_kernel<match>" : "conv3x3_wino_n_kernel");
+}
+
+}
+
+using namespace ccvpe;
+
+extern "C" int ccvpe_set_wino_n(int on) {
+  const int prev = g_wino_n ? 1 : 0;
+  g_wino_n = on != 0;
+  return prev;
+}
+
+extern "C" int ccvpe_conv3x3_wino_n_ok(const ccvpe_conv_desc* d) { return wino_n_level(d, false); }
+
+extern "C" int ccvpe_conv3x3_wino_n_f32(const ccvpe_conv_desc* d, void* stream) {
+  if (const char* why = wino_shape_refusal(d)) return fail(CCVPE_EINVAL, "conv3x3_wino_n: %s", why);
+  if (!wino_n_level(d, false)) return fail(CCVPE_EINVAL, "conv3x3_wino_n: 16 < n <= 80 only");
+  WinoNParams p{};
+  return wino_n_run<false>(d, p, (hipStream_t)stream);
+}
+
+extern "C" int ccvpe_conv3x3_wino_match1_ok(const ccvpe_conv_desc* d, int out_f32, int L) {
+  (void)out_f32;
+  if (L <= 0 || !d || L > d->n) return 0;
+  return wino_n_level(d, true);
+}
+
+extern "C" int ccvpe_conv3x3_wino_match1_f32(const ccvpe_conv_desc* d, int out_f32, const float* g, int ldg, int L, int shift, int stride,
+                                             int window_offset, float* scores, void* stream) {
+  (void)out_f32;
+  if (!d || !g || !scores) return fail(CCVPE_EINVAL, "conv3x3_wino_match1: null pointer");
+  if (L > ldg) return fail(CCVPE_EINVAL, "conv3x3_wino_match1: L > ldg");
+  if (const char* why = wino_shape_refusal(d)) return fail(CCVPE_EINVAL, "conv3x3_wino_match1: %s", why);
+  if (L <= 0 || L > d->n || !wino_n_level(d, true))
+    return fail(CCVPE_EINVAL, "conv3x3_wino_match1: needs 16 < n <= 80, n %% 4 == 0, ldd >= n + 1, 0 < L <= n");
+  WinoNParams p{};
+  p.g = g; p.scores = scores; p.ldg = ldg; p.L = L;
+  long o = (-((long)shift * stride + window_offset)) % d->n;
+  p.off = (int)(o < 0 ? o + d->n : o);
+  return wino_n_run<true>(d, p, (hipStream_t)stream);
+}
diff --git a/ccvpe_amd/csrc/conv_common.h b/ccvpe_amd/csrc/conv_common.h
--- a/ccvpe_amd/csrc/conv_common.h
+++ b/ccvpe_amd/csrc/conv_common.h
@@ -208,6 +208,8 @@
 int pwn_dispatch(const IgemmParams& p, int batch, int esz, hipStream_t stream);
 int up2_supported(int c0, int c1, int n, int kpad, int h1, int w1, int batch);
 int up2_launch(int id, const ccvpe_upconv_desc* d, hipStream_t stream);
+const char* wino_shape_refusal(const ccvpe_conv_desc* d);
+const char* wino_refusal(const ccvpe_conv_desc* d);
 bool upconv_s3q_serves(const ccvpe_upconv_desc* d);
 int upconv_s3q_launch(const ccvpe_upconv_desc* d, hipStream_t stream);
 
diff --git a/ccvpe_amd/csrc/plan.hip b/ccvpe_amd/csrc/plan.hip
--- a/ccvpe_amd/csrc/plan.hip
+++ b/ccvpe_amd/csrc/plan.hip
@@ -33,6 +33,7 @@
   static const std::unordered_map<std::string, Invoker> r = {
       CCVPE_REG(ccvpe_conv_igemm_f32), CCVPE_REG(ccvpe_conv_igemm_bf16), CCVPE_REG(ccvpe_conv_igemm_splitk_f32),
       CCVPE_REG(ccvpe_conv_igemm_splitk_bf16), CCVPE_REG(ccvpe_conv3x3_match1_bf16), CCVPE_REG(ccvpe_conv3x3_wino_f32),
+      CCVPE_REG(ccvpe_conv3x3_wino_n_f32), CCVPE_REG(ccvpe_conv3x3_wino_match1_f32),
       CCVPE_REG(ccvpe_upconv3x3_f32), CCVPE_REG(ccvpe_upconv3x3_bf16), CCVPE_REG(ccvpe_upconv3x3_s3_f32), CCVPE_REG(ccvpe_pw_s3_f32),
       CCVPE_REG(ccvpe_tail512_f32), CCVPE_REG(ccvpe_tail512_bf16), CCVPE_REG(ccvpe_stem_conv_f32), CCVPE_REG(ccvpe_stem_conv_bf16),
       CCVPE_REG(ccvpe_stem_dw_f32), CCVPE_REG(ccvpe_stem_dw_bf16),
diff --git a/ccvpe_amd/models.py b/ccvpe_amd/models.py
--- a/ccvpe_amd/models.py
+++ b/ccvpe_amd/models.py
@@ -165,6 +165,7 @@
 PACK_GRAPH = __import__("os").environ.get("CCVPE_PACK_GRAPH", "1") != "0"
 PACK_GATHER = __import__("os").environ.get("CCVPE_PACK_GATHER", "1") != "0"
 FUSE_MATCH = __import__("os").environ.get("CCVPE_FUSE_MATCH", "1") != "0"
+WINO_N_MIN_OK = 2
 FUSE_STEM = __import__("os").environ.get("CCVPE_FUSE_STEM", "1") != "0"
 EVAL_TWO_STREAMS = __import__("os").environ.get("CCVPE_EVAL_TWO_STREAMS", "1") != "0"
 
@@ -430,6 +431,9 @@
 
 def _conv_b(lv, y, batch, hw, out_f32=False):
     if (WINO and lv.u_b is not None and
+            ops.conv3x3_wino_n_ok(y, lv.n_a, lv.u_b, lv.n_b, batch=batch, in_h=hw, in_w=hw) >= WINO_N_MIN_OK):
+        return ops.conv3x3_wino_n(y, lv.n_a, lv.u_b, lv.n_b, batch=batch, in_h=hw, in_w=hw, shift=lv.b_b)
+    if (WINO and lv.u_b is not None and
             ops.conv3x3_wino_ok(y, lv.n_a, lv.u_b, lv.n_b, batch=batch, in_h=hw, in_w=hw)):
         return ops.conv3x3_wino(y, lv.n_a, lv.u_b, lv.n_b, batch=batch, in_h=hw, in_w=hw, shift=lv.b_b)
     return ops.conv_igemm(y, lv.n_a, lv.w_b, lv.n_b, batch=batch, in_h=hw, in_w=hw, kh=3, kw=3, pad=1, shift=lv.b_b,
@@ -691,7 +695,14 @@
                     to_f32 = j + 1 == pk.f32_from and y.dtype != torch.float32
                     nxt = pk.loc[j + 1]
                     L_n = gw * spec["cd"][j + 1]
-                    if (FUSE_MATCH and len(loc_shifts) == 1 and
+                    if (FUSE_MATCH and WINO and len(loc_shifts) == 1 and y.dtype == torch.float32 and lv.u_b is not None and
+                            ops.conv3x3_match1(y, lv.n_a, lv.u_b, lv.n_b, None, L_n, loc_shifts[0], strides[j + 1], nxt.ldo, batch=batch,
+                                               in_h=2 * hw, in_w=2 * hw, bias=lv.b_b, query_only=True) >= WINO_N_MIN_OK):
+                        fused = ops.conv3x3_match1(y, lv.n_a, lv.u_b, lv.n_b, gdesc[:, goff:goff + L_n], L_n, loc_shifts[0],
+                                                   strides[j + 1], nxt.ldo, batch=batch, in_h=2 * hw, in_w=2 * hw, bias=lv.b_b,
+                                                   window_offset=window_offset(self.kind, nxt.c, L_n))
+                        x = fused[1]
+                    elif (FUSE_MATCH and len(loc_shifts) == 1 and
                             ops.conv3x3_match1(y, lv.n_a, lv.w_b, lv.n_b, None, L_n, loc_shifts[0], strides[j + 1], nxt.ldo, batch=batch,
                                                in_h=2 * hw, in_w=2 * hw, bias=lv.b_b, out_f32=to_f32, query_only=True)):
                         fused = ops.conv3x3_match1(y, lv.n_a, lv.w_b, lv.n_b, gdesc[:, goff:goff + L_n], L_n, loc_shifts[0],
diff --git a/ccvpe_amd/ops.py b/ccvpe_amd/ops.py
--- a/ccvpe_amd/ops.py
+++ b/ccvpe_amd/ops.py
@@ -264,6 +264,64 @@
     return dst
 
 
+def conv3x3_wino_n_ok(src0, c0, u_packed, n, *, batch, in_h, in_w, ldd=None, ld0=None):
+    if src0.dtype != torch.float32 or u_packed is None:
+        return 0
+    ld0 = ld0 if ld0 is not None else src0.shape[-1]
+    d = _wino_desc(src0, c0, u_packed, n, batch, in_h, in_w, None, None, ldd if ldd is not None else n, ld0)
+    return int(_lib.load().ccvpe_conv3x3_wino_n_ok(ctypes.byref(d)))
+
+
+def conv3x3_wino_n(src0, c0, u_packed, n, *, batch, in_h, in_w, shift=None, dst=None, ldd=None, ld0=None):
+    lib = _lib.load()
+    for t, nm in ((src0, "src0"), (u_packed, "w"), (shift, "shift"), (dst, "dst")):
+        _chk(t, nm)
+    ld0 = ld0 if ld0 is not None else src0.shape[-1]
+    if dst is None:
+        ldd = ldd if ldd is not None else n
+        dst = _empty((batch, in_h, in_w, ldd), device=src0.device)
+    elif ldd is None:
+        ldd = dst.shape[-1]
+    d = _wino_desc(src0, c0, u_packed, n, batch, in_h, in_w, shift, dst, ldd, ld0)
+    rec = _recorder
+    ev0 = rec.begin() if rec is not None else None
+    check(lib.ccvpe_conv3x3_wino_n_f32(ctypes.byref(d), _stream()), "ccvpe_conv3x3_wino_n_f32")
+    if rec is not None:
+        m = batch * in_h * in_w
+        flops = 2.0 * m * n * 9 * c0
+        nbytes = 4.0 * (m * c0 + m * n + n * 9 * c0)
+        rec.end("conv3x3_wino_n_kernel<%d>" % (-(-n // 16)), "3x3 s1 M%d N%d K%d" % (m, n, 9 * c0), flops, nbytes, ev0)
+    return dst
+
+
+def _conv3x3_match1_f32(src0, c0, u_packed, n, g, L, shift, stride, ldo, batch, in_h, in_w, bias, window_offset, query_only):
+    lib = _lib.load()
+    if u_packed is None or u_packed.dtype != torch.float32 or src0.dtype != torch.float32:
+        if query_only:
+            return 0
+        raise ValueError("conv3x3_match1: fp32 storage needs the Winograd U pack")
+    _chk(src0, "src0")
+    _chk(u_packed, "w")
+    _chk(bias, "bias")
+    d = _wino_desc(src0, c0, u_packed, n, batch, in_h, in_w, bias, None, ldo, src0.shape[-1])
+    if query_only:
+        return int(lib.ccvpe_conv3x3_wino_match1_ok(ctypes.byref(d), 1, L))
+    if not g.is_cuda or g.dtype != torch.float32 or g.stride(-1) != 1:
+        raise ValueError("g must be an fp32 device tensor with unit inner stride")
+    scores = _empty((batch, 1, in_h, in_w), device=src0.device, dtype=torch.float32)
+    cat = _empty((batch, in_h, in_w, ldo), device=src0.device, dtype=torch.float32)
+    d.dst = _ptr(cat)
+    rec = _recorder
+    ev0 = rec.begin() if rec is not None else None
+    check(lib.ccvpe_conv3x3_wino_match1_f32(ctypes.byref(d), 1, _ptr(g), g.stride(0), L, int(shift), int(stride),
+                                            int(window_offset), _ptr(scores), _stream()), "ccvpe_conv3x3_wino_match1_f32")
+    if rec is not None:
+        m = batch * in_h * in_w
+        rec.end("conv3x3_wino_n_kernel<%d,match>" % (-(-n // 16)), "3x3+match M%d N%d K%d" % (m, n, 9 * c0), 2.0 * m * n * 9 * c0,
+                4.0 * m * c0 + 4.0 * m * ldo + 4.0 * m + 4.0 * n * 9 * c0, ev0)
+    return scores, cat
+
+
 def upconv3x3(src0, c0, w_packed, shift9, n, *, batch, h1, w1, src1=None, c1=0, act=ACT_NONE, algo_flops=None, route_only=False):
     lib = _lib.load()
     dt = _act_dtype(src0)
@@ -635,9 +693,7 @@
     lib = _lib.load()
     dt = _act_dtype(src0)
     if dt != torch.bfloat16:
-        if query_only:
-            return False
-        raise ValueError("conv3x3_match1: bf16 storage only")
+        return _conv3x3_match1_f32(src0, c0, w_packed, n, g, L, shift, stride, ldo, batch, in_h, in_w, bias, window_offset, query_only)
     _chk(src0, "src0", dt)
     _chk(w_packed, "w", dt)
     _chk(bias, "bias")
diff --git a/ccvpe_amd/plan.py b/ccvpe_amd/plan.py
--- a/ccvpe_amd/plan.py
+++ b/ccvpe_amd/plan.py
@@ -10,13 +10,13 @@
 ALIGN = 256
 
 LAUNCHES = ("ccvpe_conv_igemm_f32", "ccvpe_conv_igemm_bf16", "ccvpe_conv_igemm_splitk_f32", "ccvpe_conv_igemm_splitk_bf16",
-            "ccvpe_conv3x3_match1_bf16", "ccvpe_conv3x3_wino_f32",
+            "ccvpe_conv3x3_match1_bf16", "ccvpe_conv3x3_wino_f32", "ccvpe_conv3x3_wino_n_f32", "ccvpe_conv3x3_wino_match1_f32",
             "ccvpe_upconv3x3_f32", "ccvpe_upconv3x3_bf16", "ccvpe_upconv3x3_s3_f32", "ccvpe_pw_s3_f32", "ccvpe_tail512_f32", "ccvpe_tail512_bf16", "ccvpe_stem_conv_f32",
             "ccvpe_stem_conv_bf16", "ccvpe_stem_dw_f32", "ccvpe_stem_dw_bf16", "ccvpe_dwconv_f32", "ccvpe_dwconv_bf16", "ccvpe_mbconv_front_f32", "ccvpe_mbconv_front_bf16", "ccvpe_mbconv_front_s3_f32",
             "ccvpe_se_gate_f32", "ccvpe_ground_descriptor_f32", "ccvpe_match_level_f32", "ccvpe_match_level_bf16",
             "ccvpe_head_conv3x3_f32", "ccvpe_head_conv3x3_bf16", "ccvpe_softmax_rows_f32", "ccvpe_softmax_apply_f32", "ccvpe_cast_bf16_f32",
             "ccvpe_eval_postprocess_f32")
-QUERIES = ("ccvpe_tail512_partials", "ccvpe_conv3x3_match1_ok", "ccvpe_conv3x3_wino_ok", "ccvpe_upconv3x3_s3_ok", "ccvpe_conv_igemm_splitk_floats", "ccvpe_conv_igemm_route", "ccvpe_conv3x3_variant", "ccvpe_upconv3x3_route", "ccvpe_upconv3x3_s3_route", "ccvpe_pw_s3_ok", "ccvpe_pw_s3_route", "ccvpe_dwconv_nblk", "ccvpe_mbconv_front_nblk", "ccvpe_mbconv_front_route", "ccvpe_mbconv_front_s3_ok", "ccvpe_mbconv_band_plan", "ccvpe_stem_dw_nblk",
+QUERIES = ("ccvpe_tail512_partials", "ccvpe_conv3x3_match1_ok", "ccvpe_conv3x3_wino_ok", "ccvpe_conv3x3_wino_n_ok", "ccvpe_conv3x3_wino_match1_ok", "ccvpe_upconv3x3_s3_ok", "ccvpe_conv_igemm_splitk_floats", "ccvpe_conv_igemm_route", "ccvpe_conv3x3_variant", "ccvpe_upconv3x3_route", "ccvpe_upconv3x3_s3_route", "ccvpe_pw_s3_ok", "ccvpe_pw_s3_route", "ccvpe_dwconv_nblk", "ccvpe_mbconv_front_nblk", "ccvpe_mbconv_front_route", "ccvpe_mbconv_front_s3_ok", "ccvpe_mbconv_band_plan", "ccvpe_stem_dw_nblk",
            "ccvpe_last_error", "ccvpe_abi_version")
 
 
diff --git a/include/ccvpe_hip.h b/include/ccvpe_hip.h
--- a/include/ccvpe_hip.h
+++ b/include/ccvpe_hip.h
@@ -58,6 +58,12 @@
 int ccvpe_set_mbconv_plane_kernels(int mode);
 int ccvpe_conv3x3_wino_ok(const ccvpe_conv_desc* desc);
 int ccvpe_conv3x3_wino_f32(const ccvpe_conv_desc* desc, void* stream);
+int ccvpe_conv3x3_wino_n_ok(const ccvpe_conv_desc* desc);
+int ccvpe_conv3x3_wino_n_f32(const ccvpe_conv_desc* desc, void* stream);
+int ccvpe_conv3x3_wino_match1_ok(const ccvpe_conv_desc* desc, int out_f32, int L);
+int ccvpe_conv3x3_wino_match1_f32(const ccvpe_conv_desc* desc, int out_f32, const float* g, int ldg, int L, int shift, int stride,
+                                  int window_offset, float* scores, void* stream);
+int ccvpe_set_wino_n(int on);
 int ccvpe_conv3x3_match1_ok(const ccvpe_conv_desc* desc, int out_f32, int L);
 int ccvpe_conv3x3_match1_bf16(const ccvpe_conv_desc* desc, int out_f32, const float* g, int ldg, int L, int shift, int stride,
                               int window_offset, float* scores, void* stream);
```

Measured after the change: 2925, median of 6. 1.02x the previous value.
